# ltdoanh2004/MotionDiffusion-MoE

Hardware: AMD Instinct MI355X
Metric: denoising-steps/sec (B=32, T=196, 263-d, 8 experts) (higher is better)
Workload: dtype bf16; 1 GPU; configs[1]: model_size=small, num_experts=8, B=32/GPU, T=196, 1000-step DDPM with CFG 7.5 (cond+uncond batched as 64 rows), N_text=28, hipGraph=on, streams=1; global_batch=32, parallelism=batch-shard x1, weights replicated

## Files before the change

include/mdm_hip.h:

```cpp
#ifndef MDM_HIP_H
#define MDM_HIP_H
#include <stdint.h>

#ifdef __cplusplus
extern "C" {
#endif

enum { MDM_OK = 0, MDM_ERR_ARG = 1, MDM_ERR_LAUNCH = 2, MDM_ERR_UNSUPPORTED = 3 };
enum { MDM_OP_F32_ROW = 0, MDM_OP_F32_KSTRIDE = 1, MDM_OP_BF16_ROW = 2, MDM_OP_FP8_ROW = 3 ,
       MDM_OP_X2_ROW = 4 };
enum { MDM_ACT_NONE = 0, MDM_ACT_GELU = 1, MDM_ACT_SILU = 2, MDM_ACT_FEAT = 3,
       MDM_ACT_HEADNORM = 4,
       MDM_ACT_HEADSOFTMAX = 5 };
enum { MDM_H16_BF16 = 1, MDM_H16_F16 = 2 };
enum { MDM_PREC_BF16 = 1, MDM_PREC_F16 = 2, MDM_PREC_X3 = 3, MDM_PREC_MIXED = 4, MDM_PREC_FP8 = 5 };

typedef struct MdmOperand {
  const void* p;
  const void* p_lo;
  int64_t ld;
  int64_t gstride;
  const int32_t* gather;
  int64_t bs1, bs2;
  int32_t rpg;
// ... 266 lines not shown

int mdm_motion_fk_max_frames(void);
int mdm_motion_fk(const float* motion, const int32_t* length, const float* mean, const float* std,
                  const MdmSkeleton* skeleton, const float* offsets, int32_t offsets_per_sample, int32_t B, int32_t T,
                  int32_t F, int32_t radius, const double* weights, float* scratch, float* joints_out,
                  float* rotations_out, float* offsets_out, void* stream);

int mdm_foot_skate_max_frames(void);
int mdm_foot_skate(const float* joints, const int32_t* length, const MdmSkeleton* skeleton, const float* contact,
                   int64_t contact_stride, const float* contact_thre, double feet_thre, int32_t blend, int32_t B, int32_t T,
                   const float* rotations_in, float* joints_out, float* rotations_out, float* slide_out, int32_t* pairs_out,
                   float* scratch, void* stream);

enum { MDM_CONTROL_MAX_ITERS = 32 };
int mdm_joint_control_max_frames(int32_t feats);
int mdm_joint_loss_grad(const float* x0, const int32_t* length, const float* mean, const float* std, const float* targets,
                        const float* weights, int32_t B, int32_t T, int32_t F, float* loss_out, float* grad_out,
                        void* stream);
int mdm_joint_guidance(float* x, float* x0, const float* mask, const int32_t* length, const float* mean, const float* std,
                       const float* targets, const float* weights, int32_t B, int32_t T, int32_t F, float scale,
                       int32_t iters, const float* coef, int32_t steps, const int32_t* t_dev, int32_t t_imm,
                       void* stream);

int mdm_handshake_blend(float* x, int32_t groups, int64_t group_stride, int32_t F, int32_t nshared,
                        const int32_t* offsets, const int32_t* rows, const float* weights, void* stream);

typedef struct MdmMoeTensors {
  float* ln_w;
  float* ln_b;
  float* gate_w;
  float* gate_b;
  float* w1;
  float* b1;
  float* w2;
  float* b2;
  float* st_emb_w;
  float* st_emb_b;
  float* st_norm_w;
  float* st_norm_b;
  float* st_out_w;
  float* st_out_b;
} MdmMoeTensors;

int64_t mdm_moe_train_workspace_bytes(int32_t B, int32_t S, int32_t D, int32_t F, int32_t E, int32_t Te);
int mdm_moe_ffn_train_forward(const MdmMoeTensors* params, int32_t D, int32_t F, int32_t E, int32_t Te, int32_t De,
                              const float* eph_w, const float* eph_b, const float* x, const float* emb, int32_t B, int32_t S,
                              float dropout_p, uint64_t seed, float* out, float* lb_loss, int32_t* route_out, void* ws,
                              int64_t ws_bytes, void* stream);
int mdm_moe_ffn_train_backward(const MdmMoeTensors* params, int32_t D, int32_t F, int32_t E, int32_t Te, int32_t De,
                               const float* eph_w, const float* x, const float* emb, int32_t B, int32_t S, float dropout_p,
                               uint64_t seed, const float* dout, float* dx, float* demb, const MdmMoeTensors* grads, void* ws,
                               int64_t ws_bytes, void* stream);
int mdm_sumsq(const float* x, int64_t n, float* out, void* stream);
int mdm_adam_step(float* p, const float* g, float* m, float* v, int64_t n, float lr, float beta1, float beta2, float eps,
                  int32_t step, const float* sumsq, float max_norm, void* stream);

int mdm_xattn_gate(const float* gate, const float* adaptive_gate, int32_t D, float* out, void* stream);
int mdm_fill_i64(int64_t* dst, int64_t n, const int32_t* src_dev, void* stream);
int mdm_add_i32(int32_t* dst, int32_t delta, void* stream);

enum MdmVariant {
  MDM_VAR_DEFAULT = 0,
  MDM_VAR_GEMM_256 = 6,
  MDM_VAR_SD_UNFOLDED = 22,
  MDM_VAR_GENERIC_DH256 = 23,
  MDM_VAR_SD_FOLD_ANY = 24,
  MDM_VAR_ROUTER_CONST_E = 26,
  MDM_VAR_ROUTER_RUNTIME_E = 27,
  MDM_VAR_MLP_LDS = 34,
  MDM_VAR_TAIL_SPLIT = 35,
  MDM_VAR_X3_REG = 36,
  MDM_VAR_QKV_SPLIT = 50,
  MDM_VAR_XQ_SPLIT = 51,
  MDM_VAR_X3_ATTN_CHAIN = 52,
  MDM_VAR_X3_XATTN_CHAIN = 56,
  MDM_VAR_X3_STYLE_SPLIT = 60,
  MDM_VAR_X3_TAILS_SPLIT = 61,
  MDM_VAR_X3_F32_ROWS = 62,
  MDM_VAR_STREAM_NEVER = 63,
  MDM_VAR_STREAM_ALWAYS = 68,
  MDM_VAR_STREAM3_NEVER = 69,
  MDM_VAR_STREAM3_ALWAYS = 70
};
int mdm_set_gemm_variant(int variant);

int mdm_probe_enable(int32_t enable);
int mdm_route_dump(int32_t* buf, int64_t capacity);
int mdm_sd_fold_passes(int32_t D, int32_t H, int32_t N);
int mdm_probe_read(float* us, int32_t* rows, int32_t cap);


int64_t mdm_gru_bidir_workspace_bytes(int32_t B, int32_t H);
int mdm_gru_bidir(const float* gx, const float* w_hh, const float* b_hh, const float* h0, const int32_t* lens_dev,
                  const int32_t* lens_host, int32_t B, int32_t T, int32_t H, float* out, float* ws, int64_t ws_bytes, void* stream);
int mdm_eval_pad_rows(const float* src, int64_t ld_src, int32_t B, int32_t T, int32_t C, int32_t Cp, int32_t pad, int32_t leaky,
                      float* dst, void* stream);
int mdm_eval_ln_leaky(const float* x, int32_t M, int32_t N, const float* w, const float* b, float eps, float* y, void* stream);
int mdm_eval_matching(const float* text, const float* motion, int32_t B, int32_t D, float* dist, int32_t* rank, float* diag,
                      void* stream);
int mdm_eval_center(const float* x, int32_t N, int32_t D, float* mean, float* xc, void* stream);

const char* mdm_version(void);

#ifdef __cplusplus
}
#endif
#endif
```

motiondiffusion-moe_amd/_lib.py:

```python
from __future__ import annotations

import ctypes as C
import os

import torch

_HERE = os.path.dirname(os.path.abspath(__file__))
LIB_PATH = os.environ.get("MDM_LIB") or os.path.join(_HERE, "libmdm_hip.so")
_lib = None

OP_F32_ROW, OP_F32_KSTRIDE, OP_BF16_ROW, OP_FP8_ROW, OP_X2_ROW = 0, 1, 2, 3, 4
ACT_NONE, ACT_GELU, ACT_SILU, ACT_FEAT, ACT_HEADNORM, ACT_HEADSOFTMAX = 0, 1, 2, 3, 4, 5
H16_BF16, H16_F16 = 1, 2
PREC_BF16, PREC_F16, PREC_X3, PREC_MIXED, PREC_FP8 = 1, 2, 3, 4, 5
PRECISIONS = (PREC_BF16, PREC_F16, PREC_X3, PREC_MIXED, PREC_FP8)
PREC_NAMES = {1: "bf16", 2: "f16", 3: "bf16x3(fp32-grade)", 4: "mixed(bf16x3 + f16 expert/FFN GEMMs)",
              5: "f16 + fp8(e4m3) expert GEMMs"}


class MdmError(RuntimeError):
    pass


class Operand(C.Structure):
# ... 46 lines not shown
                ("qkv", Packed), ("qkv_b", C.c_void_p), ("hn_w", C.c_void_p), ("hn_b", C.c_void_p),
                ("feat", Packed), ("proj0", Packed), ("proj3", Packed), ("proj0_b", C.c_void_p),
                ("proj3_b", C.c_void_p), ("proj_ws", C.c_void_p), ("style", Style)]


_P2 = C.c_void_p * 2


class Layer(C.Structure):
    _fields_ = [("dual_pre_w", C.c_void_p), ("dual_pre_b", C.c_void_p), ("dual_post_w", C.c_void_p),
                ("dual_post_b", C.c_void_p), ("local", Performer), ("global_", Performer), ("skip", Packed),
                ("skip_b", C.c_void_p),
                ("ca_norm_w", C.c_void_p), ("ca_norm_b", C.c_void_p), ("ca_tnorm_w", C.c_void_p),
                ("ca_tnorm_b", C.c_void_p), ("ca_q", Packed), ("ca_k", Packed), ("ca_v", Packed),
                ("ca_q_b", C.c_void_p), ("ca_k_b", C.c_void_p), ("ca_v_b", C.c_void_p), ("ca_gvec", C.c_void_p),
                ("ca_style", Style),
                ("moe_ln_w", _P2), ("moe_ln_b", _P2), ("gate_w", _P2), ("gate_b", _P2), ("w1", Packed), ("w2", Packed),
                ("wstream", C.c_void_p), ("wstream_gs", C.c_int64), ("b1", C.c_void_p), ("b2", C.c_void_p), ("usage", _P2), ("importance", _P2), ("ffn_style", Style),
                ("sd_q", Packed), ("sd_k", Packed), ("sd_v", Packed), ("sd_out", Packed), ("sd_f1", Packed),
                ("sd_f2", Packed), ("sd_q_b", C.c_void_p), ("sd_k_b", C.c_void_p), ("sd_v_b", C.c_void_p),
                ("sd_out_b", C.c_void_p), ("sd_ln_w", C.c_void_p), ("sd_ln_b", C.c_void_p), ("sd_f1_b", C.c_void_p),
                ("sd_f2_b", C.c_void_p), ("sd_q_w32", C.c_void_p), ("sd_out_w32", C.c_void_p), ("sd_ffn_ws", C.c_void_p)]


_MODEL_PACKED = ["tmlp0", "tmlp2", "te0", "te2", "tproj", "gf_time", "gf_text", "gf_post0", "gf_post2", "text_proj",
                 "joint", "down", "up", "out"]
_MODEL_BIAS = ["tmlp0_b", "tmlp2_b", "te0_b", "te2_b", "tproj_b", "gf_time_b", "gf_text_b", "gf_post0_b", "gf_post2_b",
               "text_proj_b", "joint_b", "down_b", "up_b2", "out_b"]


class Model(C.Structure):
    _fields_ = ([(n, C.c_int32) for n in ("D", "F", "Dt", "H", "E", "L", "feats", "num_frames")]
                + [(n, Packed) for n in _MODEL_PACKED] + [(n, C.c_void_p) for n in _MODEL_BIAS]
                + [("seq_emb", C.c_void_p), ("style_eph", Packed), ("style_eph_b", C.c_void_p),
                   ("style_emb", Packed), ("style_emb_b", C.c_void_p), ("layers", C.POINTER(Layer))])


SKEL_MAX_JOINTS, SKEL_MAX_CHAINS, SKEL_MAX_CHAIN_ENTRIES = 32, 8, 48


class Skeleton(C.Structure):
    _fields_ = [("joints", C.c_int32), ("nchains", C.c_int32), ("chain_offsets", C.c_int32 * (SKEL_MAX_CHAINS + 1)),
                ("chain_joints", C.c_int32 * SKEL_MAX_CHAIN_ENTRIES), ("raw_offsets", C.c_float * (SKEL_MAX_JOINTS * 3)),
                ("face", C.c_int32 * 4), ("feet", C.c_int32 * 4), ("legs", C.c_int32 * 2)]


class TextCache(C.Structure):
    _fields_ = [("lin_at", C.c_void_p), ("sd_k", C.c_void_p), ("sd_v", C.c_void_p), ("B", C.c_int32),
                ("N", C.c_int32), ("sd_kfold", C.c_void_p), ("sd_cb", C.c_void_p), ("sd_vfold", C.c_void_p),
                ("ntok", C.c_void_p)]


class StemCache(C.Structure):
    _fields_ = [("time_table", C.c_void_p), ("gx", C.c_void_p), ("steps", C.c_int32)]


BLOCK_DUAL, BLOCK_CROSS, BLOCK_MOE, BLOCK_SDCROSS, BLOCK_LAYER = 0, 1, 2, 3, 4
NOISE_STREAM_XT = 0x7FFFFFFF
COMPOSE_MAX_K = 8
CONTROL_MAX_ITERS = 32
TAB_ROWS = 7


def lib():
    global _lib
    if _lib is None:
        if not os.path.exists(LIB_PATH):
            raise MdmError(f"{LIB_PATH} not found: build it with `python motiondiffusion-moe_amd/build.py` "
                           "(hipcc, gfx950). There is no CPU/eager fallback for the denoising path.")
        L = C.CDLL(LIB_PATH)
        L.mdm_version.restype = C.c_char_p
        for name in EXPORTS:
            if name in ("mdm_workspace_bytes", "mdm_text_head_workspace_bytes", "mdm_moe_train_workspace_bytes", "mdm_mlp_stream_elems", "mdm_gemm_stream_elems", "mdm_gemm_stream3_elems", "mdm_gemm_stream1_elems", "mdm_gemm_stream3x_elems", "mdm_gemm_stream3x_group_elems", "mdm_gru_bidir_workspace_bytes"):
                getattr(L, name).restype = C.c_int64
            elif name != "mdm_version":
                getattr(L, name).restype = C.c_int
        _lib = L
    return _lib


EXPORTS = ["mdm_version", "mdm_gemm", "mdm_fused_mlp", "mdm_mlp_stream_elems", "mdm_mlp_stream_pack", "mdm_gemm_stream_elems", "mdm_gemm_stream_pack", "mdm_gemm_stream3_elems", "mdm_gemm_stream3_pack", "mdm_gemm_stream1_elems", "mdm_gemm_stream1_pack", "mdm_gemm_stream3x_elems", "mdm_gemm_stream3x_group_elems", "mdm_gemm_stream3x_pack", "mdm_pack_bf16", "mdm_pack_f16", "mdm_pack_fp8", "mdm_workspace_bytes", "mdm_text_cache_build",
           "mdm_denoiser_forward", "mdm_stem_cache_build", "mdm_block_forward", "mdm_moe_ffn_forward", "mdm_dual_self_attn_forward", "mdm_linear_xattn_forward",
           "mdm_softmax_xattn_ffn_forward", "mdm_performer_attn_forward", "mdm_stylization_forward", "mdm_stem_embeddings",
           "mdm_cfg_posterior_step", "mdm_ddim_step", "mdm_fill_timesteps_mapped", "mdm_guided_update", "mdm_guided_update_inpaint", "mdm_composed_update", "mdm_noise_normal", "mdm_noise_normal_ids", "mdm_text_head_workspace_bytes", "mdm_text_head_forward", "mdm_motion_postprocess", "mdm_motion_features_max_frames", "mdm_motion_features", "mdm_motion_fk_max_frames", "mdm_motion_fk", "mdm_foot_skate_max_frames", "mdm_foot_skate", "mdm_joint_control_max_frames", "mdm_joint_loss_grad", "mdm_joint_guidance", "mdm_handshake_blend", "mdm_xattn_gate", "mdm_fill_i64", "mdm_add_i32", "mdm_set_gemm_variant", "mdm_probe_enable", "mdm_probe_read", "mdm_route_dump",
           "mdm_moe_train_workspace_bytes", "mdm_moe_ffn_train_forward", "mdm_moe_ffn_train_backward", "mdm_sumsq", "mdm_adam_step", "mdm_sd_fold_passes",
           "mdm_gru_bidir_workspace_bytes", "mdm_gru_bidir", "mdm_eval_pad_rows", "mdm_eval_ln_leaky", "mdm_eval_matching", "mdm_eval_center"]


def check(status: int, what: str = "mdm call"):
    if status != 0:
        names = {1: "MDM_ERR_ARG", 2: "MDM_ERR_LAUNCH", 3: "MDM_ERR_UNSUPPORTED"}
        raise MdmError(f"{what} failed: {names.get(status, status)}")


def stream_ptr() -> int:
    return torch.cuda.current_stream().cuda_stream


def ptr(t) -> int:
    return 0 if t is None else t.data_ptr()


def require_cuda(*tensors):
    for t in tensors:
        if t is not None and not t.is_cuda:
            raise MdmError("mdm HIP path needs tensors on a GPU device (no CPU fallback)")
```

motiondiffusion-moe_amd/csrc/api.hip:

```cpp
#include "gemm.h"
#include "kernels.h"

namespace mdm {
namespace {

__global__ void pack_bf16_kernel(const float* __restrict__ src, int64_t ld_src, int64_t rows, int64_t K,
                                 uint16_t* __restrict__ hi, uint16_t* __restrict__ lo, int64_t ld_dst) {
  const int64_t pairs_per_row = ld_dst >> 1;
  const int64_t total = rows * pairs_per_row;
  for (int64_t i = blockIdx.x * (int64_t)blockDim.x + threadIdx.x; i < total; i += (int64_t)gridDim.x * blockDim.x) {
    const int64_t r = i / pairs_per_row, k = (i - r * pairs_per_row) * 2;
    const float a = k < K ? src[r * ld_src + k] : 0.f;
    const float b = k + 1 < K ? src[r * ld_src + k + 1] : 0.f;
    uint32_t h, l;
    split_bf16(a, b, h, l);
    *(uint32_t*)(hi + r * ld_dst + k) = h;
    if (lo) *(uint32_t*)(lo + r * ld_dst + k) = l;
  }
}

__global__ void pack_f16_kernel(const float* __restrict__ src, int64_t ld_src, int64_t rows, int64_t K,
                                uint16_t* __restrict__ dst, int64_t ld_dst) {
  const int64_t pairs_per_row = ld_dst >> 1;
  const int64_t total = rows * pairs_per_row;
  for (int64_t i = blockIdx.x * (int64_t)blockDim.x + threadIdx.x; i < total; i += (int64_t)gridDim.x * blockDim.x) {
    const int64_t r = i / pairs_per_row, k = (i - r * pairs_per_row) * 2;
    const float a = k < K ? src[r * ld_src + k] : 0.f;
    const float b = k + 1 < K ? src[r * ld_src + k + 1] : 0.f;
    *(uint32_t*)(dst + r * ld_dst + k) = pack_f16(a, b);
  }
}

}
}

namespace mdm {
int g_variant = MDM_VAR_DEFAULT;
}

extern "C" {

int mdm_set_gemm_variant(int v) {
  switch (v) {
    case MDM_VAR_DEFAULT:
    case MDM_VAR_GEMM_256:
    case MDM_VAR_SD_UNFOLDED:
    case MDM_VAR_GENERIC_DH256:
    case MDM_VAR_SD_FOLD_ANY:
    case MDM_VAR_ROUTER_CONST_E:
    case MDM_VAR_ROUTER_RUNTIME_E:
    case MDM_VAR_MLP_LDS:
    case MDM_VAR_TAIL_SPLIT:
    case MDM_VAR_X3_REG:
    case MDM_VAR_QKV_SPLIT:
    case MDM_VAR_XQ_SPLIT:
    case MDM_VAR_X3_ATTN_CHAIN:
    case MDM_VAR_X3_XATTN_CHAIN:
    case MDM_VAR_X3_STYLE_SPLIT:
    case MDM_VAR_X3_TAILS_SPLIT:
    case MDM_VAR_X3_F32_ROWS:
    case MDM_VAR_STREAM_NEVER:
    case MDM_VAR_STREAM_ALWAYS:
    case MDM_VAR_STREAM3_NEVER:
    case MDM_VAR_STREAM3_ALWAYS:
      mdm::g_variant = v;
      return MDM_OK;
    default:
      return MDM_ERR_ARG;
  }
}

const char* mdm_version(void) { return "mdm_hip 0.1 (gfx950)"; }

int mdm_gemm(const MdmGemmDesc* d, void* stream) {
  if (!d) return MDM_ERR_ARG;
  return mdm::gemm(*d, (hipStream_t)stream);
}

int mdm_fused_mlp(const MdmMlpDesc* d, void* stream) {
  if (!d) return MDM_ERR_ARG;
  return mdm::fused_mlp(*d, (hipStream_t)stream);
}

int64_t mdm_mlp_stream_elems(int32_t G, int32_t F, int32_t Din, int32_t Dout) { return mdm::mlp_stream_elems(G, F, Din, Dout); }

int mdm_mlp_stream_pack(const float* w1, const float* w2, int32_t G, int32_t F, int32_t Din, int32_t Dout, int32_t h16,
                        uint16_t* out, void* stream) {
  return mdm::mlp_stream_pack(w1, w2, G, F, Din, Dout, h16, out, (hipStream_t)stream);
}

int64_t mdm_gemm_stream_elems(int32_t N, int32_t K) { return mdm::gemm_stream_elems(N, K); }

int mdm_gemm_stream_pack(const float* w, int32_t N, int32_t K, int32_t h16, uint16_t* out, void* stream) {
  return mdm::gemm_stream_pack(w, N, K, h16, out, (hipStream_t)stream);
}

int64_t mdm_gemm_stream1_elems(int32_t N, int32_t K) { return mdm::gemm_stream1_elems(N, K); }

int mdm_gemm_stream1_pack(const float* w, int64_t ldw, int32_t N, int32_t K, int32_t h16, uint16_t* out, void* stream) {
  return mdm::gemm_stream1_pack(w, ldw, N, K, h16, out, (hipStream_t)stream);
}

int64_t mdm_gemm_stream3x_elems(int32_t G, int32_t N, int32_t K) { return mdm::gemm_stream3x_elems(G, N, K); }

int64_t mdm_gemm_stream3x_group_elems(int32_t N, int32_t K) { return mdm::gemm_stream3x_group_elems(N, K); }

int mdm_gemm_stream3x_pack(const float* w, int64_t ldw, int32_t G, int32_t N, int32_t K, uint16_t* out, void* stream) {
  return mdm::gemm_stream3x_pack(w, ldw, G, N, K, out, (hipStream_t)stream);
}

int64_t mdm_gemm_stream3_elems(int32_t N, int32_t K) { return mdm::gemm_stream3_elems(N, K); }

int mdm_gemm_stream3_pack(const float* w, int32_t N, int32_t K, uint16_t* out, void* stream) {
  return mdm::gemm_stream3_pack(w, N, K, out, (hipStream_t)stream);
}

int mdm_pack_bf16(const float* src, int64_t ld_src, int64_t rows, int64_t K, uint16_t* hi, uint16_t* lo,
                  int64_t ld_dst, void* stream) {
  if (!src || !hi || rows < 0 || K <= 0 || ld_dst < K || (ld_dst & 31)) return MDM_ERR_ARG;
  if (rows == 0) return MDM_OK;
  const int64_t total = rows * (ld_dst >> 1);
  int blocks = (int)((total + 255) / 256);
  if (blocks > 4096) blocks = 4096;
  hipLaunchKernelGGL(mdm::pack_bf16_kernel, dim3(blocks), dim3(256), 0, (hipStream_t)stream, src, ld_src, rows, K, hi,
                     lo, ld_dst);
  MDM_RETURN_IF_LAUNCH_FAILED();
  return MDM_OK;
}

int mdm_pack_f16(const float* src, int64_t ld_src, int64_t rows, int64_t K, uint16_t* dst, int64_t ld_dst, void* stream) {
  if (!src || !dst || rows < 0 || K <= 0 || ld_dst < K || (ld_dst & 31)) return MDM_ERR_ARG;
  if (rows == 0) return MDM_OK;
  const int64_t total = rows * (ld_dst >> 1);
  int blocks = (int)((total + 255) / 256);
  if (blocks > 4096) blocks = 4096;
  hipLaunchKernelGGL(mdm::pack_f16_kernel, dim3(blocks), dim3(256), 0, (hipStream_t)stream, src, ld_src, rows, K, dst, ld_dst);
  MDM_RETURN_IF_LAUNCH_FAILED();
  return MDM_OK;
}

int mdm_fill_i64(int64_t* dst, int64_t n, const int32_t* src_dev, void* stream) {
  if (!dst || !src_dev) return MDM_ERR_ARG;
  return mdm::fill_i64(dst, n, src_dev, (hipStream_t)stream);
}

int mdm_add_i32(int32_t* dst, int32_t delta, void* stream) {
  if (!dst) return MDM_ERR_ARG;
// ... 5 lines not shown
```

motiondiffusion-moe_amd/csrc/gemm.h:

```cpp
#pragma once
#include "mdm_common.h"
#include "mdm_hip.h"

namespace mdm {

typedef MdmOperand Operand;
typedef MdmGemmDesc GemmArgs;

enum OperandKind { OP_F32_ROW = MDM_OP_F32_ROW, OP_F32_KSTRIDE = MDM_OP_F32_KSTRIDE, OP_BF16_ROW = MDM_OP_BF16_ROW, OP_X2_ROW = MDM_OP_X2_ROW };
enum Act { ACT_NONE = MDM_ACT_NONE, ACT_GELU = MDM_ACT_GELU, ACT_SILU = MDM_ACT_SILU, ACT_FEAT = MDM_ACT_FEAT, ACT_HEADNORM = MDM_ACT_HEADNORM, ACT_HEADSOFTMAX = MDM_ACT_HEADSOFTMAX };

inline GemmArgs gemm_defaults(int precision) {
  GemmArgs g = {};
  g.batch = 1;
  g.nb2 = 1;
  g.alpha = 1.f;
  g.out_scale = 1.f;
  g.r1_scale = 1.f;
  g.precision = precision;
  g.a_scale_u = 1.f;
  g.c8_scale = 1.f;
  return g;
}
inline Operand op_f32(const float* p, int64_t ld) {
  Operand o = {};
  o.p = p;
  o.ld = ld;
  o.kind = OP_F32_ROW;
  return o;
}
inline Operand op_f32_kstride(const float* p, int64_t ld) {
  Operand o = {};
  o.p = p;
  o.ld = ld;
  o.kind = OP_F32_KSTRIDE;
  return o;
}
inline Operand op_bf16(const uint16_t* hi, const uint16_t* lo, int64_t ld) {
  Operand o = {};
  o.p = hi;
  o.p_lo = lo;
  o.ld = ld;
  o.kind = OP_BF16_ROW;
  return o;
}

int gemm(const GemmArgs& a, hipStream_t stream);
bool gemm_bf16_eligible(const GemmArgs& a);
int gemm_bf16(const GemmArgs& a, hipStream_t stream);
bool gemm_bf16_256_eligible(const GemmArgs& a);
int gemm_bf16_256(const GemmArgs& a, hipStream_t stream);
bool fused_mlp_supported(const MdmMlpDesc& a);
int fused_mlp(const MdmMlpDesc& a, hipStream_t stream);
bool gemm_x3_dma_eligible(const GemmArgs& a);
int gemm_x3_dma(const GemmArgs& a, hipStream_t stream);
bool gemm_fp8_eligible(const GemmArgs& a);
int gemm_fp8(const GemmArgs& a, hipStream_t stream);
int64_t gemm_stream1_elems(int N, int K);
int gemm_stream1_pack(const float* w, int64_t ldw, int N, int K, int h16, uint16_t* out, hipStream_t stream);
bool gemm_stream1_eligible(const GemmArgs& a);
bool gemm_stream1_wanted(const GemmArgs& a);
int gemm_stream1(const GemmArgs& a, hipStream_t stream);
int64_t gemm_stream3x_elems(int G, int N, int K);
int64_t gemm_stream3x_group_elems(int N, int K);
int gemm_stream3x_pack(const float* w, int64_t ldw, int G, int N, int K, uint16_t* out, hipStream_t stream);
bool gemm_stream3x_eligible(const GemmArgs& a);
bool gemm_stream3x_wanted(const GemmArgs& a);
int gemm_stream3x(const GemmArgs& a, hipStream_t stream);
bool fused_mlp_stream_supported(const MdmMlpDesc& a);
int fused_mlp_stream(const MdmMlpDesc& a, hipStream_t stream);
struct PairTail {
  const float *pw, *pb;
  const float *sw, *sb;
  const float* sc;
  int S;
  const uint16_t* ws;
  const float* bias;
  const float* resid;
  float out_scale;
  float* out;
  const float *lw, *lb;
  uint16_t* ln16;
  const float* skip;
  float skip_scale;
  const float *l2w, *l2b;
};
bool fused_pair_style_supported(const MdmMlpDesc& a);
int fused_pair_style(const MdmMlpDesc& a, const PairTail& t, hipStream_t stream);
int64_t mlp_stream_elems(int G, int F, int Din, int Dout);
int mlp_stream_pack(const float* w1, const float* w2, int G, int F, int Din, int Dout, int h16, uint16_t* out, hipStream_t stream);
int64_t gemm_stream_elems(int N, int K);
int gemm_stream_pack(const float* w, int N, int K, int h16, uint16_t* out, hipStream_t stream);
bool style_gemm_supported(int D, int64_t M);
int64_t gemm_stream3_elems(int N, int K);
int gemm_stream3_pack(const float* w, int N, int K, uint16_t* out, hipStream_t stream);
struct StyleTail3 {
  const float *lw = nullptr, *lb = nullptr;
  float* ln_out = nullptr;
  const float* skip = nullptr;
  float skip_scale = 0.f;
  const float *l2w = nullptr, *l2b = nullptr;
  int ln_x2 = 0;
};
int style_gemm3(const float* src, int64_t M, int D, int S, const float* pw, const float* pb, const float* sw, const float* sb,
                const float* sc, const int* pos4, const uint16_t* ws3, const float* bias, const float* resid, float out_scale,
                const float* colscale, float* out, const StyleTail3& t, hipStream_t s);
int style_gemm(const void* src, int src_fmt, int64_t M, int D, int S, const float* pw, const float* pb, const float* sw, const float* sb,
               const float* sc, const int* pos4, const uint16_t* ws, const float* bias, const float* resid, float out_scale,
               const float* colscale, float* out, uint16_t* out16, int h16, hipStream_t s);

}
```

motiondiffusion-moe_amd/csrc/kernels.h:

```cpp
#pragma once
#include "mdm_common.h"

namespace mdm {

enum { TAB_SQRT_RECIP = 0, TAB_SQRT_RECIPM1 = 1, TAB_COEF1 = 2, TAB_COEF2 = 3, TAB_LOGVAR = 4, TAB_ACP = 5,
       TAB_ACP_PREV = 6, TAB_ROWS = 7 };

struct MoeGateParams {
  const float* ln_w[2];
  const float* ln_b[2];
  const float* gate_w[2];
  const float* gate_b[2];
  void* hn;
  int hn_bf16;
  float* hn_scale;
  int* top_idx;
  float* top_val;
  int* hist;
  float* uimp;
  float* usage[2];
  float* importance[2];
  const int* forced_idx;
};

int ln_chain(const float* x, int64_t M, int D, const float* w1, const float* b1, void* y1, int y1_bf, const float* w2,
             const float* b2, void* y2, int y2_bf, hipStream_t s, int x_bf = 0);
int style_in(const float* x, int64_t M, int D, int S, const float* pw, const float* pb, const float* sw,
             const float* sb, const float* sc, const int* pos4, int x_bf, void* out, int out_bf, hipStream_t s);
int to_bf16(const float* src, int64_t n, uint16_t* dst, int h16, hipStream_t s);
int f16_to_bf16x2(const uint16_t* src, int64_t n, uint16_t* hi, uint16_t* lo, hipStream_t s);
int moe_route(const float* x, int64_t M, int D, int E, const MoeGateParams& p, int* goff, int* cursor, int* perm,
              float* rowscale, int* pos4, hipStream_t s);
int head_norm(float* qkv, int64_t M, int H, int dh, const float* w, const float* b, hipStream_t s);
int den_ln(const float* num, const float* phi, int64_t M, int H, int dh, const float* w, const float* b, void* out,
           int out_bf, hipStream_t s);
int head_softmax(float* q, int64_t units, int dh, hipStream_t s);
bool perf_attn_supported(int dh, int S);
bool perf_attn_qkv_supported(int dh, int S, int H);
int perf_attn_qkv(const uint16_t* xn, const uint16_t* wqkv, int ldw, const float* bias, float alpha, uint16_t* qscratch, int h16,
                  const uint16_t* PT, int ldp, const float* hn_w, const float* hn_b, const int* len, int B, int S, int H, int dh,
                  uint16_t* out, hipStream_t s);
int perf_attn(const void* qkv, int h16, const uint16_t* PT, int ldp, const float* hn_w, const float* hn_b, const int* len, int B,
              int S, int H, int dh, uint16_t* out, hipStream_t s);
bool perf_attn256_supported(int dh, int S);
int64_t perf_attn256_scratch_bytes(int B, int H, int S);
int perf_attn256(const void* qkv, int h16, const uint16_t* PT, int ldp, const float* hn_w, const float* hn_b, const int* len,
                 int B, int S, int H, uint16_t* out, void* scratch, hipStream_t s);
bool perf_attn3_supported(int dh, int S);
int perf_attn3(const uint16_t* xh, const uint16_t* xl, const uint16_t* ph, const uint16_t* pl, int ldp, const float* hn_w,
               const float* hn_b, const int* len, int B, int S, int H, int dh, float* out, int out_x2, hipStream_t s);
bool xattn3_supported(int dh, int N);
int lin_xattn3(const uint16_t* qh, const uint16_t* ql, const float* at, int B, int S, int H, int dh, float* out, hipStream_t s);
int sd_attn3(const uint16_t* qh, const uint16_t* ql, const float* kc, const float* vc, const int32_t* ntok, int B, int S, int H,
             int dh, int N, float* out, int out_x2, hipStream_t s);
int row_softmax(float* sc, int64_t rows, int N, hipStream_t s, const int32_t* ntok = nullptr, int64_t rows_per_b = 1);
bool xattn_supported(int dh, int N);
bool lin_xattn_supported(int dh);
int sd_attn(const void* q, int q_fmt, const float* kc, const float* vc, int B, int S, int H, int dh, int N, uint16_t* out16,
            float* out32, int h16, hipStream_t s, const int32_t* ntok = nullptr);
int lin_xattn(const void* ql, int ql_fmt, const float* at, int B, int S, int H, int dh, float* out, uint16_t* out16,
              int h16, hipStream_t s);
bool lin_xattn_q_supported(int dh, int S, int H);
int lin_xattn_q(const uint16_t* xn, const uint16_t* wq, int ldw, const float* bq, const float* at, int B, int S, int H, int dh, float* out,
                uint16_t* out16, int h16, hipStream_t s);
bool sd_fold_supported(int D, int H, int N);
int sd_fold_heads_per_pass(int H, int N);
int sd_fold_passes(int H, int N);
int sd_fold(const uint16_t* x16, const uint16_t* kfold, const float* cb, const uint16_t* vfold, const float* bout,
            const float* ln_w, const float* ln_b, int B, int S, int D, int H, int N, float* out32, uint16_t* out16,
            int h16, hipStream_t s);
int col_softmax(float* k, int B, int N, int D, hipStream_t s, const int32_t* ntok = nullptr);
int sd_fold_mask_cb(float* cb, int B, int np, int hpp, int N, const int32_t* ntok, hipStream_t s);
int sinusoid(const int64_t* t, int B, int D, float* out, hipStream_t s);
int gated_mix(const float* t, const float* x, int64_t n, float* out, hipStream_t s);
int gated_mix_gather(const float* table, const int64_t* ts, int steps, const float* x, int B, int D, float* out,
                     uint16_t* out16, int h16, hipStream_t s);
int text_assemble(const float* pp, const float* ph, int B, int N0, int P, int Dt, float* xf_out, float* xf_proj,
                  hipStream_t s);
int motion_post(const float* x, const int* len, const float* mean, const float* sd, int B, int T, int feats, int J,
                int radius, const double* wts, float* raw, float* out, hipStream_t s);
bool skeleton_ok(const MdmSkeleton& s, int* parent);
int philox_normal(float* out, int64_t per_sample, int nsamples, int64_t sample0, const int64_t* sample_ids, uint64_t seed,
                  const int* stream_dev, int stream_imm, hipStream_t s);
int iota_i64(int64_t* dst, int64_t n, int64_t start, hipStream_t s);
int xattn_gate(const float* gate, const float* ag, int D, float* out, hipStream_t s);
int halve_lengths(const int* len, int B, int* out, hipStream_t s);
int fill_i64(int64_t* dst, int64_t n, const int* src, hipStream_t s);
int add_i32(int* dst, int delta, hipStream_t s);
int cfg_step(const float* x, const float* eps_c, const float* eps_u, const float* noise, int64_t n, const float* tab,
             int ts, const int* t_ptr, int t_imm, float cfg_scale, int clip, float* x_out, float* x0_out, hipStream_t s);
int ddim_step(const float* x, const float* eps, const float* noise, int64_t n, const float* tab, int ts,
              const int* t_ptr, int t_imm, float eta, int clip, float* x_out, float* x0_out, hipStream_t s);

}
```

motiondiffusion-moe_amd/csrc/model.hip:

```cpp
#include "gemm.h"
#include "kernels.h"

namespace mdm {
namespace {

#define MDM_TRY(expr)            \
  do {                           \
    int st__ = (expr);           \
    if (st__ != MDM_OK) return st__; \
  } while (0)

constexpr int PROBE_MAX = 64;
struct Probe {
  bool on = false;
  int n = 0;
  hipEvent_t a[PROBE_MAX], b[PROBE_MAX];
  int rows[PROBE_MAX];
  bool made = false;
};
Probe g_probe;
bool probe_armed() { return g_probe.on && g_probe.n < PROBE_MAX; }
int probe_begin(hipStream_t s) { return probe_armed() && hipEventRecord(g_probe.a[g_probe.n], s) != hipSuccess ? MDM_ERR_LAUNCH : MDM_OK; }
int probe_end(hipStream_t s, int rows) {
  if (!probe_armed()) return MDM_OK;
// ... 115 lines not shown
inline int fmt_mlp(const Ctx& c) { return mlp_x2(c) ? 4 : mlp16(c) ? c.h16 : 0; }

struct Act {
  void* p;
  bool bf;
  bool x2 = false;
};
inline Act act_of(const Ctx& c, float* buf) { return Act{buf, c.bf}; }
inline Act act_x2(const Ctx& c, float* buf) { return Act{buf, c.bf, x2_rows(c)}; }
inline Act act_f32(const float* buf) { return Act{(void*)buf, false}; }
inline Act act_bf16(const uint16_t* buf) { return Act{(void*)buf, true}; }

struct LinOpts {
  int act = ACT_NONE;
  float alpha = 1.f, out_scale = 1.f, r1_scale = 1.f;
  const float* R1 = nullptr;
  const float* R2 = nullptr;
  const float* colscale = nullptr;
  int r1_mod = 0;
  uint16_t* outx2 = nullptr;
};

int linear(const Ctx& c, Act A, int64_t M, int K, const MdmPacked& W, const float* bias, int N, float* out32,
           uint16_t* out16, const LinOpts& o = LinOpts()) {
  GemmArgs g = gd(c);
  if (A.bf) {
    g.A.p = A.p, g.A.ld = K, g.A.kind = OP_BF16_ROW;
    g.precision = 1;
  } else {
    g.A = op_f32((const float*)A.p, K);
    if (A.x2) g.A.kind = OP_X2_ROW;
  }
  g.W = packed(W);
  g.w_stream = A.bf ? W.ws : nullptr;
  g.M = (int)M, g.N = N, g.K = K;
  g.C = out32, g.C16 = out16, g.ldc = N;
  g.Cx2 = o.outx2;
  g.bias = bias;
  g.act = o.act, g.alpha = o.alpha, g.out_scale = o.out_scale;
  g.R1 = o.R1, g.ldr1 = N, g.r1_scale = o.r1_scale, g.r1_mod = o.r1_mod;
  g.R2 = o.R2, g.ldr2 = N;
  g.colscale = o.colscale;
  if (A.bf && !gemm_bf16_eligible(g)) return MDM_ERR_UNSUPPORTED;
  return gemm(g, c.s);
}
int linear_to_act(const Ctx& c, Act A, int64_t M, int K, const MdmPacked& W, const float* bias, int N, float* buf,
                  const LinOpts& o = LinOpts()) {
  return linear(c, A, M, K, W, bias, N, c.bf ? nullptr : buf, c.bf ? (uint16_t*)buf : nullptr, o);
}

inline Operand heads(Operand o, int64_t bs1, int64_t bs2) { o.bs1 = bs1, o.bs2 = bs2; return o; }
GemmArgs per_head(const Ctx& c, Operand A, Operand W, int M, int N, int K, int64_t ldc, int64_t c_bs1, int64_t c_bs2) {
  GemmArgs g = gd(c);
  g.A = A, g.W = W;
  g.M = M, g.N = N, g.K = K;
  g.batch = c.B * c.m->H, g.nb2 = c.m->H;
  g.ldc = ldc, g.c_bs1 = c_bs1, g.c_bs2 = c_bs2;
  return g;
}

GemmArgs planes_gemm(const Ctx& c, Act A, const MdmPacked& W, const float* bias, int N, uint16_t* hi, uint16_t* lo) {
  const int K = c.m->D;
  GemmArgs g = gd(c);
  g.A = op_f32((const float*)A.p, K);
  if (A.x2) g.A.kind = OP_X2_ROW;
  g.W = packed(W);
  g.M = (int)c.M, g.N = N, g.K = K;
  g.bias = bias;
  g.C16 = hi, g.C16_lo = lo, g.ldc = N;
  return g;
}

enum class StylePath { FUSED16, FUSED3, FUSED3_TAIL, SPLIT };
StylePath style_path(const Ctx& c, const MdmStyle& st, bool src16, bool out16, bool tail) {
  const int D = c.m->D;
  if (c.bf && st.out_ws && style_gemm_supported(D, c.M)) return StylePath::FUSED16;
  if (x3_flow(c) && !src16 && !out16 && st.out_ws3 && g_variant != MDM_VAR_X3_STYLE_SPLIT && style_gemm_supported(D, c.M))
    return tail && g_variant != MDM_VAR_X3_TAILS_SPLIT ? StylePath::FUSED3_TAIL : StylePath::FUSED3;
  return StylePath::SPLIT;
}

int style_apply(const Ctx& c, const MdmStyle& st, const float* src, const float* pw, const float* pb, const int* pos4,
                const float* sc, float* tmp, const float* resid, float out_scale, const float* colscale, float* out,
                uint16_t* out16 = nullptr, bool src_bf16 = false, const StyleTail3* t3 = nullptr) {
  const int D = c.m->D;
  const StylePath path = style_path(c, st, src_bf16, out16 != nullptr, t3 != nullptr);
  switch (path) {
    case StylePath::FUSED16:
      return style_gemm(src, src_bf16 ? c.h16 : 0, c.M, D, c.S, pw, pb, st.norm_w, st.norm_b, sc, pos4, st.out_ws, st.out_b, resid,
                        out_scale, colscale, out, out16, c.h16, c.s);
    case StylePath::FUSED3:
    case StylePath::FUSED3_TAIL:
      return style_gemm3(src, c.M, D, c.S, pw, pb, st.norm_w, st.norm_b, sc, pos4, st.out_ws3, st.out_b, resid, out_scale, colscale, out,
                         path == StylePath::FUSED3_TAIL ? *t3 : StyleTail3(), c.s);
    case StylePath::SPLIT: {
      MDM_TRY(style_in(src, c.M, D, c.S, pw, pb, st.norm_w, st.norm_b, sc, pos4, src_bf16 ? c.h16 : 0, tmp, fmt16(c), c.s));
      LinOpts o;
      o.out_scale = out_scale, o.R1 = resid, o.colscale = colscale;
      return linear(c, act_of(c, tmp), c.M, D, st.out, st.out_b, D, out, out16, o);
    }
  }
}

MdmMlpDesc proj_pair_desc(const Ctx& c, const MdmPerformer& p) {
  const int D = c.m->D;
  MdmMlpDesc f = {};
  f.X = (const uint16_t*)c.w.t4, f.ldx = D, f.M = (int)c.M, f.Din = D, f.F = D, f.Dout = D;
  f.b1 = p.proj0_b, f.b2 = p.proj3_b, f.wstream = p.proj_ws, f.wstream_gs = 2 * (int64_t)D * D;
  f.r1_scale = 1.f, f.C16 = (uint16_t*)c.w.t4, f.ldc = D, f.h16 = c.h16;
  return f;
}
enum class ProjPath { PAIR_TAIL, PAIR, LINEARS_X2, LINEARS };
ProjPath proj_path(const Ctx& c, const MdmPerformer& p) {
  if (c.bf && p.proj_ws) {
    const MdmMlpDesc f = proj_pair_desc(c, p);
    if (p.style.out_ws && g_variant != MDM_VAR_TAIL_SPLIT && fused_pair_style_supported(f)) return ProjPath::PAIR_TAIL;
    if (fused_mlp_stream_supported(f)) return ProjPath::PAIR;
  }
  return x2_rows(c) ? ProjPath::LINEARS_X2 : ProjPath::LINEARS;
}

enum class PerfCore { CORE3, CORE256, CORE16_QKV, CORE16, CHAIN };
PerfCore perf_core_path(const Ctx& c, const MdmPerformer& p, bool xn16) {
  const int D = c.m->D, H = c.m->H, dh = D / H;
  if (c.bf && g_variant != MDM_VAR_GENERIC_DH256 && perf_attn256_supported(dh, c.S) &&
      perf_attn256_scratch_bytes(c.B, H, c.S) <= c.M * 2 * D * (int64_t)sizeof(float))
    return PerfCore::CORE256;
  if (c.bf && perf_attn_supported(dh, c.S))
    return xn16 && g_variant != MDM_VAR_QKV_SPLIT && perf_attn_qkv_supported(dh, c.S, H) ? PerfCore::CORE16_QKV : PerfCore::CORE16;
  if (x3_flow(c) && !xn16 && g_variant != MDM_VAR_X3_ATTN_CHAIN && perf_attn3_supported(dh, c.S) && D % 32 == 0 && p.qkv.lo &&
      p.feat.lo && (c.M * 3 * D) % 8 == 0)
    return PerfCore::CORE3;
  return PerfCore::CHAIN;
}

int performer(const Ctx& c, const MdmPerformer& p, const float* x, Act xn, const float* sc, float* out,
              const StyleTail3& pt = StyleTail3()) {
  const MdmModel& m = *c.m;
  const int D = m.D, H = m.H, dh = D / H, mf = dh;
  const Work& w = c.w;
  LinOpts qo;
  qo.alpha = 0.1f;
  Act att = act_of(c, w.t4);
  switch (perf_core_path(c, p, xn.bf)) {
    case PerfCore::CORE3: {
      uint16_t* const xh = (uint16_t*)w.qkv;
      uint16_t* const xl = xh + c.M * 3 * D;
      GemmArgs g = planes_gemm(c, xn, p.qkv, p.qkv_b, 3 * D, xh, xl);
      g.alpha = 0.1f, g.act = ACT_HEADNORM, g.hn_w = p.hn_w, g.hn_b = p.hn_b, g.hn_l2_tiles = 2 * H;
      MDM_TRY(gemm(g, c.s));
      MDM_TRY(perf_attn3(xh, xl, p.feat.hi, p.feat.lo, (int)p.feat.ld, p.hn_w, p.hn_b, c.len, c.B, c.S, H, dh, w.t4, c.x2 ? 1 : 0, c.s));
      att.x2 = c.x2;
      break;
    }
    case PerfCore::CORE256:
      MDM_TRY(linear(c, xn, c.M, D, p.qkv, p.qkv_b, 3 * D, nullptr, (uint16_t*)w.qkv, qo));
      MDM_TRY(perf_attn256(w.qkv, c.h16, p.feat.hi, (int)p.feat.ld, p.hn_w, p.hn_b, c.len, c.B, c.S, H, (uint16_t*)w.t4, w.phi, c.s));
      break;
    case PerfCore::CORE16_QKV:
      MDM_TRY(perf_attn_qkv((const uint16_t*)xn.p, p.qkv.hi, (int)p.qkv.ld, p.qkv_b, 0.1f, (uint16_t*)w.qkv, c.h16, p.feat.hi,
                            (int)p.feat.ld, p.hn_w, p.hn_b, c.len, c.B, c.S, H, dh, (uint16_t*)w.t4, c.s));
      break;
    case PerfCore::CORE16:
      MDM_TRY(linear(c, xn, c.M, D, p.qkv, p.qkv_b, 3 * D, nullptr, (uint16_t*)w.qkv, qo));
      MDM_TRY(perf_attn(w.qkv, c.h16, p.feat.hi, (int)p.feat.ld, p.hn_w, p.hn_b, c.len, c.B, c.S, H, dh, (uint16_t*)w.t4, c.s));
      break;
    case PerfCore::CHAIN: {
      MDM_TRY(linear(c, xn, c.M, D, p.qkv, p.qkv_b, 3 * D, w.qkv, nullptr, qo));
      MDM_TRY(head_norm(w.qkv, c.M, H, dh, p.hn_w, p.hn_b, c.s));
      const bool f16p = c.bf && c.h16 == MDM_H16_F16 && !p.feat.lo;
      Operand P = packed(p.feat);
      if (f16p) {
        const int64_t pn = (int64_t)mf * p.feat.ld;
// ... 33 lines not shown
      t.ws = p.style.out_ws, t.bias = p.style.out_b, t.resid = x, t.out_scale = 0.1f, t.out = out;
      t.lw = pt.lw, t.lb = pt.lb, t.ln16 = (uint16_t*)pt.ln_out, t.skip = pt.skip, t.skip_scale = pt.skip_scale, t.l2w = pt.l2w, t.l2b = pt.l2b;
      return fused_pair_style(proj_pair_desc(c, p), t, c.s);
    }
    case ProjPath::PAIR:
      MDM_TRY(fused_mlp_stream(proj_pair_desc(c, p), c.s));
      break;
    case ProjPath::LINEARS_X2: {
      LinOpts o;
      o.act = ACT_GELU, o.outx2 = (uint16_t*)w.t2;
      MDM_TRY(linear(c, att, c.M, D, p.proj0, p.proj0_b, D, nullptr, nullptr, o));
      MDM_TRY(linear(c, Act{w.t2, false, true}, c.M, D, p.proj3, p.proj3_b, D, w.t4, nullptr));
      break;
    }
    case ProjPath::LINEARS: {
      LinOpts o;
      o.act = ACT_GELU;
      MDM_TRY(linear_to_act(c, att, c.M, D, p.proj0, p.proj0_b, D, w.t2, o));
      MDM_TRY(linear_to_act(c, act_of(c, w.t2), c.M, D, p.proj3, p.proj3_b, D, w.t4));
      break;
    }
  }
  const bool tail3 = !c.bf && (pt.ln_out || pt.skip);
  return style_apply(c, p.style, w.t4, p.post_w, p.post_b, nullptr, sc, w.t2, x, 0.1f, nullptr, out, nullptr, c.bf,
                     tail3 ? &pt : nullptr);
}

enum class DualTail { NONE, T16, T3 };
DualTail dual_tail_path(const Ctx& c, const MdmLayer& l) {
  if (proj_path(c, l.local) == ProjPath::PAIR_TAIL && proj_path(c, l.global) == ProjPath::PAIR_TAIL) return DualTail::T16;
  if (style_path(c, l.local.style, false, false, true) == StylePath::FUSED3_TAIL &&
      style_path(c, l.global.style, false, false, true) == StylePath::FUSED3_TAIL)
    return DualTail::T3;
  return DualTail::NONE;
}

int dual_block(const Ctx& c, const MdmLayer& l, const float* x, const uint16_t* x16, const float* sc4, float* out,
               const float* next_w = nullptr, const float* next_b = nullptr) {
  const int D = c.m->D;
  const Work& w = c.w;
  const int64_t scs = (int64_t)c.B * 2 * D;
  const int xnf = fmt_xn(c);
  const Act xa = c.bf ? act_bf16(x16) : act_f32(x);
  LinOpts so;
  so.act = ACT_GELU;
  switch (dual_tail_path(c, l)) {
    case DualTail::T16:
    case DualTail::T3: {
      MDM_TRY(linear(c, xa, c.M, D, l.skip, l.skip_b, D, w.f1, nullptr, so));
      MDM_TRY(ln_chain(x, c.M, D, l.dual_pre_w, l.dual_pre_b, w.t1, 0, l.local.pre_w, l.local.pre_b, w.t3, xnf, c.s));
      StyleTail3 pt;
      pt.lw = l.global.pre_w, pt.lb = l.global.pre_b, pt.ln_out = w.t3, pt.ln_x2 = c.x2;
      MDM_TRY(performer(c, l.local, w.t1, act_x2(c, w.t3), sc4 + 0 * scs, w.t5, pt));
      StyleTail3 bt;
      bt.skip = w.f1, bt.skip_scale = 0.1f, bt.lw = l.dual_post_w, bt.lb = l.dual_post_b;
      if (next_w) bt.l2w = next_w, bt.l2b = next_b, bt.ln_out = w.t2, bt.ln_x2 = c.x2;
      return performer(c, l.global, w.t5, act_x2(c, w.t3), sc4 + 1 * scs, out, bt);
    }
    case DualTail::NONE: {
      MDM_TRY(ln_chain(x, c.M, D, l.dual_pre_w, l.dual_pre_b, w.t1, 0, l.local.pre_w, l.local.pre_b, w.t3, xnf, c.s));
      const bool normed = proj_path(c, l.local) == ProjPath::PAIR_TAIL;
      StyleTail3 pt;
      if (normed) pt.lw = l.global.pre_w, pt.lb = l.global.pre_b, pt.ln_out = w.t3;
      MDM_TRY(performer(c, l.local, w.t1, act_x2(c, w.t3), sc4 + 0 * scs, w.t5, pt));
      if (!normed) MDM_TRY(ln_chain(w.t5, c.M, D, l.global.pre_w, l.global.pre_b, w.t3, xnf, nullptr, nullptr, nullptr, 0, c.s));
      MDM_TRY(performer(c, l.global, w.t5, act_x2(c, w.t3), sc4 + 1 * scs, w.t1));
      so.R1 = w.t1, so.r1_scale = 0.1f;
      MDM_TRY(linear(c, xa, c.M, D, l.skip, l.skip_b, D, w.t3, nullptr, so));
      return ln_chain(w.t3, c.M, D, l.dual_post_w, l.dual_post_b, out, 0, next_w, next_b, next_w ? w.t2 : nullptr, xnf, c.s);
    }
  }
}

enum class XattnPath { CORE3, CORE_Q, CORE, CHAIN };
XattnPath lin_xattn_path(const Ctx& c, const MdmLayer& l) {
  const int D = c.m->D, H = c.m->H, dh = D / H;
  if (c.bf && lin_xattn_supported(dh) && !(dh == 256 && g_variant == MDM_VAR_GENERIC_DH256))
    return g_variant != MDM_VAR_XQ_SPLIT && D == 512 && lin_xattn_q_supported(dh, c.S, H) ? XattnPath::CORE_Q : XattnPath::CORE;
  if (x3_flow(c) && g_variant != MDM_VAR_X3_XATTN_CHAIN && xattn3_supported(dh, 1) && l.ca_q.lo && D % 32 == 0 && (c.M * D) % 8 == 0)
    return XattnPath::CORE3;
  return XattnPath::CHAIN;
}

int cross_block(const Ctx& c, const MdmLayer& l, const float* at, const float* x, const float* sc, float* out,
                bool pre_normed = false) {
  const MdmModel& m = *c.m;
  const int D = m.D, H = m.H, dh = D / H;
  const Work& w = c.w;
  if (!pre_normed) MDM_TRY(ln_chain(x, c.M, D, l.ca_norm_w, l.ca_norm_b, w.t2, fmt_xn(c), nullptr, nullptr, nullptr, 0, c.s));
  bool y16 = false;
  switch (lin_xattn_path(c, l)) {
    case XattnPath::CORE3: {
      uint16_t* const qh = (uint16_t*)w.t3;
      uint16_t* const ql = qh + c.M * D;
      GemmArgs g = planes_gemm(c, act_x2(c, w.t2), l.ca_q, l.ca_q_b, D, qh, ql);
      g.act = ACT_HEADSOFTMAX;
      MDM_TRY(gemm(g, c.s));
      MDM_TRY(lin_xattn3(qh, ql, at, c.B, c.S, H, dh, w.t4, c.s));
      break;
    }
    case XattnPath::CORE_Q:
      MDM_TRY(lin_xattn_q((const uint16_t*)w.t2, l.ca_q.hi, (int)l.ca_q.ld, l.ca_q_b, at, c.B, c.S, H, dh, nullptr, (uint16_t*)w.t4,
                          c.h16, c.s));
      y16 = true;
      break;
    case XattnPath::CORE:
      MDM_TRY(linear(c, act_x2(c, w.t2), c.M, D, l.ca_q, l.ca_q_b, D, nullptr, (uint16_t*)w.t3));
      MDM_TRY(lin_xattn(w.t3, c.h16, at, c.B, c.S, H, dh, nullptr, (uint16_t*)w.t4, c.h16, c.s));
      y16 = true;
      break;
    case XattnPath::CHAIN: {
      MDM_TRY(linear(c, act_x2(c, w.t2), c.M, D, l.ca_q, l.ca_q_b, D, w.t3, nullptr));
      MDM_TRY(head_softmax(w.t3, c.M * H, dh, c.s));
      GemmArgs g = per_head(c, heads(op_f32(w.t3, D), (int64_t)c.S * D, dh), heads(op_f32(at, dh), (int64_t)H * dh * dh, (int64_t)dh * dh),
                            c.S, dh, dh, D, (int64_t)c.S * D, dh);
      g.C = w.t4;
      MDM_TRY(gemm(g, c.s));
      break;
    }
  }
  return style_apply(c, l.ca_style, w.t4, nullptr, nullptr, nullptr, sc, w.t2, x, 1.f, l.ca_gvec, out, nullptr, y16);
}

GemmArgs expert_gemm(const Ctx& c, const void* A, int K, const MdmPacked& W, const float* bias, int N) {
  GemmArgs g = gd(c);
  if (c.fp8) {
    g.A.p = A, g.A.ld = K, g.A.kind = MDM_OP_FP8_ROW;
    g.W.p = W.hi, g.W.ld = W.ld, g.W.kind = MDM_OP_FP8_ROW, g.w_scale = (const float*)W.lo;
  } else if (mlp16(c)) {
    g.A.p = A, g.A.ld = K, g.A.kind = OP_BF16_ROW, g.precision = 1;
    g.W = packed(W);
  } else {
    g.A = op_f32((const float*)A, K);
    if (mlp_x2(c)) g.A.kind = OP_X2_ROW;
    g.W = packed(W);
  }
  g.W.bs1 = (int64_t)N * W.ld;
  g.goff = c.w.goff, g.ngroups = 2 * c.m->E;
  g.M = (int)(4 * c.M), g.N = N, g.K = K;
  g.bias = bias, g.bias_bs = N;
  g.ldc = N;
  if (mlp_x2(c) && W.ws) g.w_stream = W.ws, g.w_stream_gs = gemm_stream3x_group_elems(N, K);
  return g;
}
enum class MoePath { FP8, FUSED, GROUPED };
MoePath moe_path(const Ctx& c, const MdmMlpDesc& f) {
  if (c.fp8) return MoePath::FP8;
  return mlp16(c) && fused_mlp_supported(f) ? MoePath::FUSED : MoePath::GROUPED;
}

int moe_block(const Ctx& c, const MdmLayer& l, const float* x, const float* sc, const int* forced, float* out,
              uint16_t* out16, int32_t* route_out = nullptr) {
  const MdmModel& m = *c.m;
  const int D = m.D, F = m.F, E = m.E;
  const Work& w = c.w;
  MoeGateParams p = {};
  for (int b = 0; b < 2; ++b) {
    p.ln_w[b] = l.moe_ln_w[b], p.ln_b[b] = l.moe_ln_b[b];
    p.gate_w[b] = l.gate_w[b], p.gate_b[b] = l.gate_b[b];
    p.usage[b] = l.usage[b], p.importance[b] = l.importance[b];
  }
  p.hn = w.hn, p.hn_bf16 = c.fp8 ? 3 : fmt_mlp(c), p.hn_scale = w.hn_scale, p.top_idx = w.top_idx, p.top_val = w.top_val, p.hist = w.hist, p.uimp = w.uimp, p.forced_idx = forced;
  MDM_TRY(moe_route(x, c.M, D, E, p, w.goff, w.cursor, w.perm, w.rowscale, w.pos4, c.s));
  if (route_out && hipMemcpyAsync(route_out, w.top_idx, 4 * c.M * sizeof(int32_t), hipMemcpyDeviceToDevice, c.s) != hipSuccess)
    return MDM_ERR_LAUNCH;
  MdmMlpDesc f = {};
  f.X = (const uint16_t*)w.hn, f.ldx = D, f.gather = w.perm;
  f.M = (int)(4 * c.M), f.Din = D, f.F = F, f.Dout = D;
  f.goff = w.goff, f.ngroups = 2 * E;
  f.w1 = l.w1.hi, f.ldw1 = l.w1.ld, f.w1_gs = (int64_t)F * l.w1.ld, f.b1 = l.b1, f.b1_gs = F;
  f.w2 = l.w2.hi, f.ldw2 = l.w2.ld, f.w2_gs = (int64_t)D * l.w2.ld, f.b2 = l.b2, f.b2_gs = D;
  f.rowscale = w.rowscale, f.r1_scale = 1.f;
  f.C = w.y2, f.ldc = D;
  f.h16 = c.h16;
  f.wstream = l.wstream, f.wstream_gs = l.wstream_gs;
  switch (moe_path(c, f)) {
    case MoePath::FP8: {
      const float HS = 8.f;
      GemmArgs g1 = expert_gemm(c, w.hn, D, l.w1, l.b1, F);
      g1.A.gather = w.perm, g1.a_scale = w.hn_scale, g1.act = ACT_GELU, g1.C8 = (uint8_t*)w.hid, g1.c8_scale = HS;
      MDM_TRY(gemm(g1, c.s));
      GemmArgs g2 = expert_gemm(c, w.hid, F, l.w2, l.b2, D);
      g2.a_scale_u = 1.f / HS, g2.rowscale = w.rowscale, g2.C16 = (uint16_t*)w.y2;
      MDM_TRY(gemm(g2, c.s));
      return style_apply(c, l.ffn_style, w.y2, nullptr, nullptr, w.pos4, sc, w.t2, x, 1.f, nullptr, out, out16, true);
    }
    case MoePath::FUSED: {
      if (c.bf) f.C = nullptr, f.C16 = (uint16_t*)w.y2;
      MDM_TRY(probe_begin(c.s));
      MDM_TRY(fused_mlp(f, c.s));
      MDM_TRY(probe_end(c.s, f.M));
      return style_apply(c, l.ffn_style, w.y2, nullptr, nullptr, w.pos4, sc, w.t2, x, 1.f, nullptr, out, out16, c.bf);
    }
    case MoePath::GROUPED: {
      MDM_TRY(probe_begin(c.s));
      GemmArgs g1 = expert_gemm(c, w.hn, D, l.w1, l.b1, F);
      g1.A.gather = w.perm, g1.act = ACT_GELU;
      if (mlp16(c)) g1.C16 = (uint16_t*)w.hid;
      else if (mlp_x2(c)) g1.Cx2 = (uint16_t*)w.hid;
      else g1.C = w.hid;
      MDM_TRY(gemm(g1, c.s));
      GemmArgs g2 = expert_gemm(c, w.hid, F, l.w2, l.b2, D);
      g2.rowscale = w.rowscale, g2.C = w.y2;
      MDM_TRY(gemm(g2, c.s));
      MDM_TRY(probe_end(c.s, (int)(4 * c.M)));
      return style_apply(c, l.ffn_style, w.y2, nullptr, nullptr, w.pos4, sc, w.t2, x, 1.f, nullptr, out, out16, false);
    }
  }
}

int sd_fold_policy(int D, int H, int N) {
  if (!sd_fold_supported(D, H, N)) return 0;
  const int np = sd_fold_passes(H, N);
  return (np <= 2 || g_variant == MDM_VAR_SD_FOLD_ANY) ? np : 0;
}

struct SdFold {
  const uint16_t* kfold = nullptr;
  const float* cb = nullptr;
  const uint16_t* vfold = nullptr;
};

enum class SdPath { FOLD_PAIR, FOLD, CORE3, CORE, CHAIN };
SdPath sd_path(const Ctx& c, const MdmLayer& l, const SdFold& fold, const MdmMlpDesc& f) {
  const int D = c.m->D, H = c.m->H, dh = D / H, N = c.N;
  if (c.bf && fold.kfold && g_variant != MDM_VAR_SD_UNFOLDED && sd_fold_policy(D, H, N) > 0)
    return l.sd_ffn_ws && c.S >= 128 && fused_mlp_stream_supported(f) ? SdPath::FOLD_PAIR : SdPath::FOLD;
  if (x3_flow(c) && g_variant != MDM_VAR_X3_XATTN_CHAIN && xattn3_supported(dh, N) && l.sd_q.lo && D % 32 == 0 && (c.M * D) % 8 == 0)
    return SdPath::CORE3;
  if (c.bf && xattn_supported(dh, N) && !(dh == 256 && g_variant == MDM_VAR_GENERIC_DH256)) return SdPath::CORE;
  return SdPath::CHAIN;
}

int sd_ffn(const Ctx& c, const MdmLayer& l, const float* x, float* out, uint16_t* out16) {
  const int D = c.m->D;
  const Work& w = c.w;
  const bool h = mlp16(c), x2 = mlp_x2(c);
  LinOpts o1;
  o1.act = ACT_GELU;
  if (x2) o1.outx2 = (uint16_t*)w.f1;
  MDM_TRY(linear(c, Act{w.t4, h, x2}, c.M, D, l.sd_f1, l.sd_f1_b, 4 * D, (h || x2) ? nullptr : w.f1, h ? (uint16_t*)w.f1 : nullptr, o1));
  LinOpts o;
  o.R1 = x, o.R2 = w.t3;
  return linear(c, Act{w.f1, h, x2}, c.M, 4 * D, l.sd_f2, l.sd_f2_b, D, out, out16, o);
}

// ... 6 lines not shown
  f.X = (const uint16_t*)w.t4, f.ldx = D, f.M = (int)c.M, f.Din = D, f.F = 4 * D, f.Dout = D;
  f.b1 = l.sd_f1_b, f.b2 = l.sd_f2_b, f.wstream = l.sd_ffn_ws, f.wstream_gs = 8 * (int64_t)D * D;
  f.R1 = x, f.ldr1 = D, f.r1_scale = 1.f, f.R2 = w.t3, f.ldr2 = D;
  f.C = out, f.C16 = out16, f.ldc = D, f.h16 = c.h16;
  const SdPath path = sd_path(c, l, fold, f);
  const Act xa = c.bf ? act_bf16(x16) : act_f32(x);
  LinOpts qo;
  qo.alpha = 1.f / sqrtf((float)dh);
  Act att = act_of(c, w.t2);
  switch (path) {
    case SdPath::FOLD_PAIR:
    case SdPath::FOLD:
      MDM_TRY(sd_fold(x16, fold.kfold, fold.cb, fold.vfold, l.sd_out_b, l.sd_ln_w, l.sd_ln_b, c.B, c.S, D, H, N, w.t3,
                      (uint16_t*)w.t4, c.h16, c.s));
      return path == SdPath::FOLD_PAIR ? fused_mlp_stream(f, c.s) : sd_ffn(c, l, x, out, out16);
    case SdPath::CORE3: {
      uint16_t* const qh = (uint16_t*)w.t1;
      uint16_t* const ql = qh + c.M * D;
      GemmArgs g = planes_gemm(c, act_f32(x), l.sd_q, l.sd_q_b, D, qh, ql);
      g.alpha = qo.alpha;
      MDM_TRY(gemm(g, c.s));
      MDM_TRY(sd_attn3(qh, ql, kc, vc, c.ntok, c.B, c.S, H, dh, N, w.t2, c.x2 ? 1 : 0, c.s));
      att.x2 = c.x2;
      break;
    }
    case SdPath::CORE:
      MDM_TRY(linear(c, xa, c.M, D, l.sd_q, l.sd_q_b, D, nullptr, (uint16_t*)w.t1, qo));
      MDM_TRY(sd_attn(w.t1, c.h16, kc, vc, c.B, c.S, H, dh, N, (uint16_t*)w.t2, nullptr, c.h16, c.s, c.ntok));
      break;
    case SdPath::CHAIN: {
      MDM_TRY(linear(c, xa, c.M, D, l.sd_q, l.sd_q_b, D, w.t1, nullptr, qo));
      GemmArgs g = per_head(c, heads(op_f32(w.t1, D), (int64_t)c.S * D, dh), heads(op_f32(kc, D), (int64_t)N * D, dh), c.S, N, dh,
                            N, (int64_t)H * c.S * N, (int64_t)c.S * N);
      g.C = w.scr;
      MDM_TRY(gemm(g, c.s));
      MDM_TRY(row_softmax(w.scr, c.M * H, N, c.s, c.ntok, (int64_t)H * c.S));
      GemmArgs pv = per_head(c, heads(op_f32(w.scr, N), (int64_t)H * c.S * N, (int64_t)c.S * N),
                             heads(op_f32_kstride(vc, D), (int64_t)N * D, dh), c.S, dh, N, D, (int64_t)c.S * D, dh);
      pv.C = c.bf ? nullptr : w.t2, pv.C16 = c.bf ? (uint16_t*)w.t2 : nullptr;
      MDM_TRY(gemm(pv, c.s));
      break;
    }
  }
  MDM_TRY(linear(c, att, c.M, D, l.sd_out, l.sd_out_b, D, w.t3, nullptr));
  MDM_TRY(ln_chain(w.t3, c.M, D, l.sd_ln_w, l.sd_ln_b, w.t4, fmt_mlp(c), nullptr, nullptr, nullptr, 0, c.s));
  return sd_ffn(c, l, x, out, out16);
}

const float* tc_at(const MdmModel& m, const MdmTextCache& tc, int layer) {
  const int dh = m.D / m.H;
  return tc.lin_at + (int64_t)layer * tc.B * m.H * dh * dh;
}
const float* tc_k(const MdmModel& m, const MdmTextCache& tc, int layer) {
  return tc.sd_k + (int64_t)layer * tc.B * tc.N * m.D;
}
const float* tc_v(const MdmModel& m, const MdmTextCache& tc, int layer) {
  return tc.sd_v + (int64_t)layer * tc.B * tc.N * m.D;
}
SdFold tc_fold(const MdmModel& m, const MdmTextCache& tc, int layer) {
  SdFold f;
  if (tc.sd_kfold && tc.sd_cb && tc.sd_vfold) {
    const int64_t np = sd_fold_passes(m.H, tc.N);
    f.kfold = tc.sd_kfold + (int64_t)layer * tc.B * np * 128 * m.D;
    f.cb = tc.sd_cb + (int64_t)layer * tc.B * np * 128;
    f.vfold = tc.sd_vfold + (int64_t)layer * tc.B * np * m.D * 128;
  }
  return f;
}

int decoder_layer(const Ctx& c, int layer, const MdmTextCache& tc, float* x, uint16_t* x16, float* y, uint16_t* y16,
                  const float* sc4, const int* forced, float* trace, int32_t* route_out = nullptr) {
  const MdmModel& m = *c.m;
  const MdmLayer& l = m.layers[layer];
  const int64_t scs = (int64_t)c.B * 2 * m.D, n = c.M * m.D;
  auto dump = [&](int slot, const float* p) -> int {
    if (!trace) return MDM_OK;
    return hipMemcpyAsync(trace + (int64_t)slot * n, p, n * sizeof(float), hipMemcpyDeviceToDevice, c.s) == hipSuccess
               ? MDM_OK
               : MDM_ERR_LAUNCH;
  };
  if (!c.bf) x16 = y16 = nullptr;
  MDM_TRY(dual_block(c, l, x, x16, sc4, y, l.ca_norm_w, l.ca_norm_b));
  MDM_TRY(dump(0, y));
  MDM_TRY(cross_block(c, l, tc_at(m, tc, layer), y, sc4 + 2 * scs, x, true));
  MDM_TRY(dump(1, x));
  MDM_TRY(moe_block(c, l, x, sc4 + 3 * scs, forced, y, y16, route_out));
  MDM_TRY(dump(2, y));
  MDM_TRY(sdcross_block(c, l, tc_k(m, tc, layer), tc_v(m, tc, layer), y, y16, x, x16, tc_fold(m, tc, layer)));
  return dump(3, x);
}

int stem_time_branch(const Ctx& c, const int64_t* timesteps, int B, float* dst) {
  const MdmModel& m = *c.m;
  const int D = m.D, Te = 4 * D;
  const Work& w = c.w;
  LinOpts silu_o;
  silu_o.act = ACT_SILU;
  MDM_TRY(sinusoid(timesteps, B, D, w.s_a, c.s));
  MDM_TRY(linear(c, act_f32(w.s_a), B, D, m.tmlp0, m.tmlp0_b, 2 * D, w.s_b, nullptr, silu_o));
  MDM_TRY(linear(c, act_f32(w.s_b), B, 2 * D, m.tmlp2, m.tmlp2_b, D, w.s_a, nullptr));
  MDM_TRY(linear(c, act_f32(w.s_a), B, D, m.te0, m.te0_b, Te, w.s_b, nullptr, silu_o));
  MDM_TRY(linear(c, act_f32(w.s_b), B, Te, m.te2, m.te2_b, Te, w.s_c, nullptr));
  MDM_TRY(linear(c, act_f32(w.s_c), B, Te, m.tproj, m.tproj_b, D, w.s_a, nullptr));
  return linear(c, act_f32(w.s_a), B, D, m.gf_time, m.gf_time_b, D, dst, nullptr);
}

int stem_text_branch(const Ctx& c, const float* xf_proj, int B, float* dst) {
  const MdmModel& m = *c.m;
  const float* tp = xf_proj;
  if (m.Dt != m.D) {
    if (!m.text_proj.hi) return MDM_ERR_ARG;
    MDM_TRY(linear(c, act_f32(xf_proj), B, m.Dt, m.text_proj, m.text_proj_b, m.D, c.w.s_c, nullptr));
    tp = c.w.s_c;
  }
  return linear(c, act_f32(tp), B, m.D, m.gf_text, m.gf_text_b, m.D, dst, nullptr);
}

int stem_embeddings(const Ctx& c, const int64_t* timesteps, const float* xf_proj, const MdmStemCache* sc_cache,
                    float* emb_out, float* sc_out) {
  const MdmModel& m = *c.m;
  const int D = m.D, Te = 4 * D, B = c.B, nblk = 8 * m.L;
  const Work& w = c.w;
  LinOpts silu_o;
  silu_o.act = ACT_SILU;
  float* mix = w.s_b;
  if (sc_cache && sc_cache->time_table && sc_cache->gx) {
    MDM_TRY(gated_mix_gather(sc_cache->time_table, timesteps, sc_cache->steps, sc_cache->gx, B, D, c.bf ? nullptr : mix,
                             c.bf ? (uint16_t*)mix : nullptr, c.h16, c.s));
  } else {
    MDM_TRY(stem_time_branch(c, timesteps, B, w.s_b));
    MDM_TRY(stem_text_branch(c, xf_proj, B, w.s_a));
    MDM_TRY(gated_mix(w.s_b, w.s_a, (int64_t)B * D, w.s_c, c.s));
    if (c.bf) {
      MDM_TRY(to_bf16(w.s_c, (int64_t)B * D, (uint16_t*)w.s_b, c.h16, c.s));
    } else {
      mix = w.s_c;
    }
  }
  MDM_TRY(linear_to_act(c, act_of(c, mix), B, D, m.gf_post0, m.gf_post0_b, D, w.s_a, silu_o));
  float* emb = emb_out ? emb_out : w.emb;
  MDM_TRY(linear(c, act_of(c, w.s_a), B, D, m.gf_post2, m.gf_post2_b, D, emb, c.bf ? (uint16_t*)w.s_c : nullptr));
  MDM_TRY(linear_to_act(c, c.bf ? act_bf16((uint16_t*)w.s_c) : act_f32(emb), B, D, m.style_eph, m.style_eph_b, nblk * Te,
                        w.e1, silu_o));
  GemmArgs g = gd(c);
  if (c.bf) {
    g.A.p = w.e1, g.A.ld = (int64_t)nblk * Te, g.A.kind = OP_BF16_ROW, g.precision = 1;
  } else {
    g.A = op_f32(w.e1, (int64_t)nblk * Te);
  }
  g.A.bs1 = Te;
  g.W = packed(m.style_emb);
  g.W.bs1 = (int64_t)2 * D * m.style_emb.ld;
  g.M = B, g.N = 2 * D, g.K = Te;
  g.batch = nblk, g.nb2 = 1;
  g.bias = m.style_emb_b, g.bias_bs = 2 * D;
  g.C = sc_out, g.ldc = 2 * D, g.c_bs1 = (int64_t)B * 2 * D;
  return gemm(g, c.s);
}

int check_model(const MdmModel* m) {
  if (!m || !m->layers || m->D <= 0 || m->H <= 0 || m->D % m->H || m->L <= 0 || m->E < 2 || m->E > 16) return MDM_ERR_ARG;
  const int dh = m->D / m->H;
  if (dh != 16 && dh != 32 && dh != 64 && dh != 128 && dh != 256) return MDM_ERR_UNSUPPORTED;
  if (m->D > 1024 || m->Dt > 1024 || (m->D & 3) || (m->F & 3)) return MDM_ERR_UNSUPPORTED;
  return MDM_OK;
}

}
}
// ... 239 lines not shown
                                  int64_t ws_bytes, int32_t precision, void* stream) {
  return mdm_block_forward(m, layer, MDM_BLOCK_SDCROSS, tc, h, sc4, len, B, S, out, ws, ws_bytes, nullptr, precision, stream);
}
int mdm_performer_attn_forward(const MdmModel* m, int32_t layer, int32_t which, const float* h, const float* sc,
                               const int32_t* len, int32_t B, int32_t S, float* out, void* ws, int64_t ws_bytes,
                               int32_t precision, void* stream) {
  MDM_TRY(check_model(m));
  if (!h || !sc || !len || !out || !ws || B <= 0 || S <= 0 || layer < 0 || layer >= 2 * m->L || which < 0 || which > 1)
    return MDM_ERR_ARG;
  Ctx c = {};
  c.m = m, c.s = (hipStream_t)stream, c.B = B, c.S = S, c.M = (int64_t)B * S, c.len = len, c.N = 1;
  if (!set_precision(c, m, precision)) return MDM_ERR_UNSUPPORTED;
  c.w = carve(*m, B, S, 1, ws);
  if (c.w.bytes > ws_bytes) return MDM_ERR_ARG;
  const MdmLayer& l = m->layers[layer];
  const MdmPerformer& p = which ? l.global : l.local;
  MDM_TRY(ln_chain(h, c.M, m->D, p.pre_w, p.pre_b, c.w.t3, fmt16(c), nullptr, nullptr, nullptr, 0, c.s));
  return performer(c, p, h, act_of(c, c.w.t3), sc, out);
}

int mdm_stylization_forward(const MdmStyle* st, const float* h, const float* sc, int32_t B, int32_t S, int32_t D,
                            float* tmp, float* out, int32_t precision, void* stream) {
  if (!st || !h || !sc || !tmp || !out || B <= 0 || S <= 0) return MDM_ERR_ARG;
  MdmModel fake = {};
  fake.D = D;
  Ctx c = {};
  fake.F = D;
  c.m = &fake, c.s = (hipStream_t)stream, c.B = B, c.S = S, c.M = (int64_t)B * S;
  if (!set_precision(c, &fake, precision)) return MDM_ERR_UNSUPPORTED;
  return style_apply(c, *st, h, nullptr, nullptr, nullptr, sc, tmp, nullptr, 1.f, nullptr, out);
}

int64_t mdm_text_head_workspace_bytes(int32_t B, int32_t N0, int32_t P, int32_t Hs, int32_t Dt) {
  if (B <= 0 || N0 < 0 || P < 0 || Hs <= 0 || Dt <= 0) return -1;
  const int64_t fl = (int64_t)B * N0 * Hs + (int64_t)P * Hs + (int64_t)B * N0 * Dt + (int64_t)P * Dt;
  return ((fl * 4 + 255) & ~(int64_t)255) + 1024;
}

int mdm_text_head_forward(const float* hidden, const float* prompts, const float* ln_w, const float* ln_b,
                          const MdmPacked* w, const float* bias, int32_t B, int32_t N0, int32_t P, int32_t Hs,
                          int32_t Dt, float* xf_out, float* xf_proj, void* ws, int64_t ws_bytes, int32_t precision,
                          void* stream) {
  if (!ln_w || !ln_b || !w || !w->hi || !xf_out || !xf_proj || !ws || B <= 0 || N0 < 0 || P < 0 || N0 + P <= 0 ||
      (N0 > 0 && !hidden) || (P > 0 && !prompts))
    return MDM_ERR_ARG;
  if (precision != 1 && precision != 3) return MDM_ERR_ARG;
  if (precision == 3 && !w->lo) return MDM_ERR_ARG;
  if (ws_bytes < mdm_text_head_workspace_bytes(B, N0, P, Hs, Dt)) return MDM_ERR_ARG;
  hipStream_t s = (hipStream_t)stream;
  Bump b(ws);
  float* lnh = b.take<float>((int64_t)B * N0 * Hs);
  float* lnp = b.take<float>((int64_t)P * Hs);
  float* ph = b.take<float>((int64_t)B * N0 * Dt);
  float* pp = b.take<float>((int64_t)P * Dt);
  MdmModel fake = {};
  Ctx c = {};
  c.m = &fake, c.s = s, c.prec = precision, c.bf = false, c.mix = false, c.h16 = MDM_H16_BF16;
  LinOpts o;
  o.act = ACT_GELU;
  if (N0 > 0) {
    MDM_TRY(ln_chain(hidden, (int64_t)B * N0, Hs, ln_w, ln_b, lnh, 0, nullptr, nullptr, nullptr, 0, s));
    MDM_TRY(linear(c, act_f32(lnh), (int64_t)B * N0, Hs, *w, bias, Dt, ph, nullptr, o));
  }
  if (P > 0) {
    MDM_TRY(ln_chain(prompts, P, Hs, ln_w, ln_b, lnp, 0, nullptr, nullptr, nullptr, 0, s));
    MDM_TRY(linear(c, act_f32(lnp), P, Hs, *w, bias, Dt, pp, nullptr, o));
  }
  return text_assemble(pp, ph, B, N0, P, Dt, xf_out, xf_proj, s);
}

int mdm_motion_postprocess(const float* motion, const int32_t* length, const float* mean, const float* std, int32_t B,
                           int32_t T, int32_t feats, int32_t joints, int32_t radius, const double* weights,
                           float* scratch, float* joints_out, void* stream) {
  if (!motion || !mean || !std || !scratch || !joints_out || B <= 0 || T <= 0 || joints < 1 || radius < 0 ||
      (radius > 0 && !weights))
    return MDM_ERR_ARG;
  if (feats < 4 + 3 * (joints - 1)) return MDM_ERR_ARG;
  return motion_post(motion, length, mean, std, B, T, feats, joints, radius, weights, scratch, joints_out,
                     (hipStream_t)stream);
}

int mdm_sd_fold_passes(int32_t D, int32_t H, int32_t N) { return sd_fold_policy(D, H, N); }

int mdm_route_dump(int32_t* buf, int64_t capacity) {
  if (buf && capacity <= 0) return MDM_ERR_ARG;
  g_route_dump = buf, g_route_cap = buf ? capacity : 0;
  return MDM_OK;
}

int mdm_probe_enable(int32_t enable) {
  if (enable && !g_probe.made) {
    for (int i = 0; i < PROBE_MAX; ++i)
      if (hipEventCreate(&g_probe.a[i]) != hipSuccess || hipEventCreate(&g_probe.b[i]) != hipSuccess) return MDM_ERR_LAUNCH;
    g_probe.made = true;
  }
  g_probe.on = enable != 0;
  if (enable) g_probe.n = 0;
  return MDM_OK;
}

int mdm_probe_read(float* us, int32_t* rows, int32_t cap) {
  const int n = g_probe.n;
  for (int i = 0; i < n && i < cap; ++i) {
    if (hipEventSynchronize(g_probe.b[i]) != hipSuccess) return -1;
    float ms = 0.f;
    if (hipEventElapsedTime(&ms, g_probe.a[i], g_probe.b[i]) != hipSuccess) return -1;
    if (us) us[i] = ms * 1e3f;
    if (rows) rows[i] = g_probe.rows[i];
  }
  return n;
}

int mdm_cfg_posterior_step(const float* x, const float* eps_c, const float* eps_u, const float* noise, int64_t n,
                           const float* tab, int32_t steps, const int32_t* t_dev, int32_t t_imm, float cfg_scale,
                           int32_t clip_denoised, float* x_out, float* x0_out, void* stream) {
  if (steps <= 0 || (!t_dev && (t_imm < 0 || t_imm >= steps))) return MDM_ERR_ARG;
  return cfg_step(x, eps_c, eps_u, noise, n, tab, steps, t_dev, t_imm, cfg_scale, clip_denoised, x_out, x0_out,
                  (hipStream_t)stream);
}

int mdm_ddim_step(const float* x, const float* eps, const float* noise, int64_t n, const float* tab, int32_t steps,
                  const int32_t* t_dev, int32_t t_imm, float eta, int32_t clip_denoised, float* x_out, float* x0_out,
                  void* stream) {
  if (steps <= 0 || (!t_dev && (t_imm < 0 || t_imm >= steps))) return MDM_ERR_ARG;
  return ddim_step(x, eps, noise, n, tab, steps, t_dev, t_imm, eta, clip_denoised, x_out, x0_out, (hipStream_t)stream);
}

int mdm_xattn_gate(const float* gate, const float* adaptive_gate, int32_t D, float* out, void* stream) {
  if (!gate || !adaptive_gate || !out || D <= 0) return MDM_ERR_ARG;
  return xattn_gate(gate, adaptive_gate, D, out, (hipStream_t)stream);
}

}
```

motiondiffusion-moe_amd/csrc/rowwise.hip:

```cpp
#include "kernels.h"
#include "row.h"

namespace mdm {
namespace {

template <int NE, bool VEC, int FMT>
__device__ __forceinline__ void ln_chain_rows(const float* __restrict__ x, bool x_h, int64_t M, int D, const float* w1,
                                              const float* b1, void* y1, int y1_h, const float* w2, const float* b2,
                                              void* y2, int y2_h) {
  const int lane = threadIdx.x & 63;
  Row<NE, VEC> ww1, bb1, ww2, bb2;
  ww1.load(w1, D, lane), bb1.load(b1, D, lane);
  if (w2) ww2.load(w2, D, lane), bb2.load(b2, D, lane);
  for (int64_t row = 2 * (blockIdx.x * (int64_t)WPB + (threadIdx.x >> 6)); row < M; row += 2 * (int64_t)gridDim.x * WPB) {
    const bool two = row + 1 < M;
    Row<NE, VEC> r, q;
    if (x_h) {
      r.template load_h16<FMT>((const uint16_t*)x + row * D, D, lane);
      q.template load_h16<FMT>((const uint16_t*)x + (two ? row + 1 : row) * D, D, lane);
    } else {
      r.load(x + row * D, D, lane);
      q.load(x + (two ? row + 1 : row) * D, D, lane);
    }
    r.layernorm(ww1, bb1, D, lane);
    q.layernorm(ww1, bb1, D, lane);
    if (y1) {
      r.template store_mode<FMT>(y1, row, D, lane, y1_h);
      if (two) q.template store_mode<FMT>(y1, row + 1, D, lane, y1_h);
    }
    if (w2) {
      r.layernorm(ww2, bb2, D, lane);
      q.layernorm(ww2, bb2, D, lane);
      r.template store_mode<FMT>(y2, row, D, lane, y2_h);
      if (two) q.template store_mode<FMT>(y2, row + 1, D, lane, y2_h);
    }
  }
}
template <int NE, bool VEC>
__global__ __launch_bounds__(256) void ln_chain_kernel(const float* __restrict__ x, int x_bf, int64_t M, int D,
                                                       const float* w1, const float* b1, void* y1, int y1_bf,
                                                       const float* w2, const float* b2, void* y2, int y2_bf) {
  const int m1 = y1_bf == 4 ? 2 : (y1_bf != 0), m2 = y2_bf == 4 ? 2 : (y2_bf != 0);
  if (((x_bf | y1_bf | y2_bf) & 3) == 2) {
    ln_chain_rows<NE, VEC, 2>(x, x_bf != 0, M, D, w1, b1, y1, m1, w2, b2, y2, m2);
  } else {
    ln_chain_rows<NE, VEC, 1>(x, x_bf != 0, M, D, w1, b1, y1, m1, w2, b2, y2, m2);
  }
}

template <int NE, bool VEC, int FMT>
__device__ __forceinline__ void style_in_rows(const float* __restrict__ x, int64_t M, int D, int S, const float* pw,
                                              const float* pb, const float* sw, const float* sb,
                                              const float* __restrict__ sc, const int* __restrict__ pos4, bool x_h,
                                              void* __restrict__ out, bool out_h) {
  const int lane = threadIdx.x & 63;
  Row<NE, VEC> pww, pbb, sww, sbb;
  if (pw) pww.load(pw, D, lane), pbb.load(pb, D, lane);
  sww.load(sw, D, lane), sbb.load(sb, D, lane);
  for (int64_t row = blockIdx.x * (int64_t)WPB + (threadIdx.x >> 6); row < M; row += (int64_t)gridDim.x * WPB) {
    const float* scb = sc + (row / S) * 2 * (int64_t)D;
    Row<NE, VEC> r, scale, shift;
    scale.load(scb, D, lane);
    shift.load(scb + D, D, lane);
    if (pos4) {
      const int p0 = pos4[row * 4 + 0], p1 = pos4[row * 4 + 1], p2 = pos4[row * 4 + 2], p3 = pos4[row * 4 + 3];
      Row<NE, VEC> a, b, c, d;
      if (x_h) {
        const uint16_t* xh = (const uint16_t*)x;
        a.template load_h16<FMT>(xh + (int64_t)p0 * D, D, lane);
        b.template load_h16<FMT>(xh + (int64_t)p1 * D, D, lane);
        c.template load_h16<FMT>(xh + (int64_t)p2 * D, D, lane);
        d.template load_h16<FMT>(xh + (int64_t)p3 * D, D, lane);
      } else {
        a.load(x + (int64_t)p0 * D, D, lane);
        b.load(x + (int64_t)p1 * D, D, lane);
        c.load(x + (int64_t)p2 * D, D, lane);
        d.load(x + (int64_t)p3 * D, D, lane);
      }
#pragma unroll
      for (int j = 0; j < NE; ++j) r.e[j] = ((a.e[j] + b.e[j]) + (c.e[j] + d.e[j])) * 0.5f;
    } else {
      if (x_h) {
        r.template load_h16<FMT>((const uint16_t*)x + row * D, D, lane);
// ... 92 lines not shown
              v2 = pe, i2 = e;
            }
          }
        }
        if (!(v2 >= 0.f)) {
          i2 = i1 == 0 ? 1 : 0;
          v1 = v2 = __int_as_float(0x7fc00000);
        }
      }
      if (lane == 0) {
        const int64_t o = ((int64_t)br * M + row) * 2;
        p.top_idx[o] = i1, p.top_idx[o + 1] = i2;
        p.top_val[o] = v1, p.top_val[o + 1] = v2;
        atomicAdd(&s_hist[br * E + i1], 1);
        atomicAdd(&s_hist[br * E + i2], 1);
        atomicAdd(&s_usage[br * E + i1], 1.f);
        atomicAdd(&s_imp[br * E + i1], v1);
        atomicAdd(&s_imp[br * E + i2], v2);
      }
    }
  }
  __syncthreads();
  if (threadIdx.x < 2 * E) {
    const int g = threadIdx.x;
    p.hist[blockIdx.x * 32 + g] = s_hist[g];
    p.uimp[blockIdx.x * 64 + g] = s_usage[g];
    p.uimp[blockIdx.x * 64 + 32 + g] = s_imp[g];
  }
}

template <int NV, bool FAST, int EX = 0, int HNF = -1>
__global__ __launch_bounds__(256) void moe_gate16_kernel(const float* __restrict__ x, int64_t M, int D_rt, int E_rt,
                                                         MoeGateParams p) {
  const int E = EX > 0 ? EX : E_rt;
  const int hnf = HNF >= 0 ? HNF : p.hn_bf16;
  constexpr int D = 64 * NV;
  extern __shared__ __attribute__((aligned(16))) float gsm[];
  float* gw = gsm;
  float* lnw = gsm + 2 * E * D;
  float* lnb = lnw + 2 * D;
  int* s_hist = (int*)(lnb + 2 * D);
  float* s_usage = (float*)(s_hist + 32);
  float* s_imp = s_usage + 32;
  const int l16 = threadIdx.x & 15;
  const int64_t tpb = 16;
  const int64_t stride = (int64_t)gridDim.x * tpb;
  auto load_x = [&](int64_t base, f32x4(&r)[NV]) {
    const int64_t row = base + (threadIdx.x >> 4);
    const int64_t rc = row < M ? row : M - 1;
#pragma unroll
    for (int c = 0; c < NV; ++c) r[c] = *(const f32x4*)(x + rc * D + 4 * (l16 + 16 * c));
  };
  f32x4 vn[NV];
  if constexpr (NV <= 8)
    if (blockIdx.x * tpb < M) load_x(blockIdx.x * tpb, vn);
#pragma unroll
  for (int br = 0; br < 2; ++br) {
    const float* src = p.gate_w[br];
    const int n4 = E * D / 4;
    for (int i0 = threadIdx.x; i0 < n4; i0 += 4 * 256) {
      f32x4 t[4];
#pragma unroll
      for (int j = 0; j < 4; ++j)
        if (i0 + 256 * j < n4) t[j] = *(const f32x4*)(src + 4 * (i0 + 256 * j));
#pragma unroll
      for (int j = 0; j < 4; ++j)
        if (i0 + 256 * j < n4) *(f32x4*)(gw + br * E * D + 4 * (i0 + 256 * j)) = t[j];
    }
  }
  for (int i = threadIdx.x; i < D / 4; i += 256) {
    const f32x4 w0 = *(const f32x4*)(p.ln_w[0] + 4 * i), w1 = *(const f32x4*)(p.ln_w[1] + 4 * i);
    const f32x4 b0 = *(const f32x4*)(p.ln_b[0] + 4 * i), b1 = *(const f32x4*)(p.ln_b[1] + 4 * i);
    *(f32x4*)(lnw + 4 * i) = w0, *(f32x4*)(lnw + D + 4 * i) = w1;
    *(f32x4*)(lnb + 4 * i) = b0, *(f32x4*)(lnb + D + 4 * i) = b1;
  }
  if (threadIdx.x < 32) s_hist[threadIdx.x] = 0, s_usage[threadIdx.x] = 0.f, s_imp[threadIdx.x] = 0.f;
  __syncthreads();
  for (int64_t base = blockIdx.x * tpb; base < M; base += stride) {
    const int64_t row = base + (threadIdx.x >> 4);
    const bool ok = row < M;
    const int64_t rc = ok ? row : M - 1;
    if constexpr (NV > 8) load_x(base, vn);
    f32x4 v[NV];
    float s = 0.f;
#pragma unroll
    for (int c = 0; c < NV; ++c) {
      v[c] = vn[c];
      s += v[c][0] + v[c][1] + v[c][2] + v[c][3];
    }
    if constexpr (NV <= 8)
      if (base + stride < M) load_x(base + stride, vn);
    const float mean = group_sum<16>(s) / D;
    float q = 0.f;
#pragma unroll
    for (int c = 0; c < NV; ++c) {
      v[c] = (f32x4){v[c][0] - mean, v[c][1] - mean, v[c][2] - mean, v[c][3] - mean};
      q += v[c][0] * v[c][0] + v[c][1] * v[c][1] + v[c][2] * v[c][2] + v[c][3] * v[c][3];
    }
    const float rstd = rsqrtf(group_sum<16>(q) / D + 1e-5f);
#pragma unroll
    for (int br = 0; br < 2; ++br) {
      float logit[16];
#pragma unroll
      for (int e = 0; e < 16; ++e) logit[e] = 0.f;
      float amax = 0.f;
#pragma unroll
      for (int c = 0; c < NV; ++c) {
        const int k = 4 * (l16 + 16 * c);
        const f32x4 w = *(const f32x4*)(lnw + br * D + k), b = *(const f32x4*)(lnb + br * D + k);
        const f32x4 h = {v[c][0] * rstd * w[0] + b[0], v[c][1] * rstd * w[1] + b[1], v[c][2] * rstd * w[2] + b[2],
                         v[c][3] * rstd * w[3] + b[3]};
        amax = fmaxf(amax, fmaxf(fmaxf(fabsf(h[0]), fabsf(h[1])), fmaxf(fabsf(h[2]), fabsf(h[3]))));
        if constexpr (HNF >= 0) {
          if constexpr (HNF == 1 || HNF == 2) {
            *(uint2*)((uint16_t*)p.hn + ((int64_t)br * M + rc) * D + k) = make_uint2(pack_h16(HNF, h[0], h[1]), pack_h16(HNF, h[2], h[3]));
          } else if constexpr (HNF == 0) {
            *(f32x4*)((float*)p.hn + ((int64_t)br * M + rc) * D + k) = h;
          } else if constexpr (HNF == 4) {
            static_assert(D % 32 == 0, "lane pairs of store_x2_4p hold k and k ^ 4 of one 32-column block");
            store_x2_4p((uint16_t*)p.hn + ((int64_t)br * M + rc) * 2 * D, k, h[0], h[1], h[2], h[3]);
          }
        } else if (ok && p.hn_bf16 != 3) {
          if (p.hn_bf16 == 4) {
            store_x2_4((uint16_t*)p.hn + ((int64_t)br * M + row) * 2 * D, k, h[0], h[1], h[2], h[3]);
          } else if (p.hn_bf16 == 2) {
            *(uint2*)((uint16_t*)p.hn + ((int64_t)br * M + row) * D + k) = make_uint2(pack_h16(2, h[0], h[1]), pack_h16(2, h[2], h[3]));
          } else if (p.hn_bf16) {
            *(uint2*)((uint16_t*)p.hn + ((int64_t)br * M + row) * D + k) = make_uint2(pack_h16(1, h[0], h[1]), pack_h16(1, h[2], h[3]));
          } else {
            *(f32x4*)((float*)p.hn + ((int64_t)br * M + row) * D + k) = h;
          }
        }
#pragma unroll
        for (int e = 0; e < 16; ++e)
          if (e < E) {
            const f32x4 g = *(const f32x4*)(gw + (br * E + e) * D + k);
            if constexpr (FAST) {
              logit[e] = __builtin_fmaf(h[3], g[3], __builtin_fmaf(h[2], g[2], __builtin_fmaf(h[1], g[1], __builtin_fmaf(h[0], g[0], logit[e]))));
            } else {
              logit[e] += h[0] * g[0] + h[1] * g[1] + h[2] * g[2] + h[3] * g[3];
            }
          }
        if constexpr (EX > 0 && HNF >= 0) __builtin_amdgcn_sched_barrier(0);
      }
      if (hnf == 3) {
        amax = group_max<16>(amax);
        const float scale = amax > 0.f ? amax * (1.f / 448.f) : 1.f, inv = 1.f / scale;
#pragma unroll
        for (int c = 0; c < NV; ++c) {
          const int k = 4 * (l16 + 16 * c);
          const f32x4 w = *(const f32x4*)(lnw + br * D + k), b = *(const f32x4*)(lnb + br * D + k);
          uint32_t q = 0;
          q = __builtin_amdgcn_cvt_pk_fp8_f32((v[c][0] * rstd * w[0] + b[0]) * inv, (v[c][1] * rstd * w[1] + b[1]) * inv, q, false);
          q = __builtin_amdgcn_cvt_pk_fp8_f32((v[c][2] * rstd * w[2] + b[2]) * inv, (v[c][3] * rstd * w[3] + b[3]) * inv, q, true);
          if (HNF >= 0 || ok) *(uint32_t*)((uint8_t*)p.hn + ((int64_t)br * M + (HNF >= 0 ? rc : row)) * D + k) = q;
        }
        if (ok && l16 == 0) p.hn_scale[(int64_t)br * M + row] = scale;
      }
      float mx = -INFINITY, mine = -INFINITY;
#pragma unroll
      for (int e = 0; e < 16; ++e) {
        if (e < E) {
          logit[e] = group_sum<16>(logit[e]) + p.gate_b[br][e];
          mx = fmaxf(mx, logit[e]);
          mine = (l16 == e) ? logit[e] : mine;
        }
      }
      const float den = group_sum<16>(l16 < E ? expf(mine - mx) : 0.f);
      int i1 = 0, i2 = 1;
      float l1 = -INFINITY, l2 = -INFINITY;
      if (p.forced_idx) {
        i1 = min(max(p.forced_idx[((int64_t)br * M + rc) * 2 + 0], 0), E - 1);
        i2 = min(max(p.forced_idx[((int64_t)br * M + rc) * 2 + 1], 0), E - 1);
#pragma unroll
        for (int e = 0; e < 16; ++e) {
          l1 = e == i1 ? logit[e] : l1;
          l2 = e == i2 ? logit[e] : l2;
        }
      } else {
#pragma unroll
        for (int e = 0; e < 16; ++e) {
          if (e < E) {
            if (logit[e] > l1) {
              l2 = l1, i2 = i1;
              l1 = logit[e], i1 = e;
            } else if (logit[e] > l2) {
              l2 = logit[e], i2 = e;
            }
          }
        }
        if (i2 == i1) i2 = i1 == 0 ? 1 : 0;
      }
      const float v1 = expf(l1 - mx) / den, v2 = expf(l2 - mx) / den;
      if (ok && l16 == 0) {
        const int64_t o = ((int64_t)br * M + row) * 2;
        p.top_idx[o] = i1, p.top_idx[o + 1] = i2;
        p.top_val[o] = v1, p.top_val[o + 1] = v2;
        atomicAdd(&s_hist[br * E + i1], 1);
        atomicAdd(&s_hist[br * E + i2], 1);
        atomicAdd(&s_usage[br * E + i1], 1.f);
        atomicAdd(&s_imp[br * E + i1], v1);
        atomicAdd(&s_imp[br * E + i2], v2);
      }
    }
  }
  __syncthreads();
  if (threadIdx.x < 2 * E) {
    const int g = threadIdx.x;
    p.hist[blockIdx.x * 32 + g] = s_hist[g];
    p.uimp[blockIdx.x * 64 + g] = s_usage[g];
    p.uimp[blockIdx.x * 64 + 32 + g] = s_imp[g];
  }
}

__global__ __launch_bounds__(1024) void moe_offsets_kernel(const int* __restrict__ hist_part,
                                                            const float* __restrict__ uimp_part, int nparts, int E,
                                                            int* __restrict__ goff, int* __restrict__ cursor,
                                                            MoeGateParams p) {
  __shared__ int sh[32][33];
  __shared__ float su[32][33], si[32][33];
  __shared__ int tot[32];
  const int g = threadIdx.x & 31, c = threadIdx.x >> 5, G = 2 * E;
  int h = 0;
  float u = 0.f, im = 0.f;
  if (g < G) {
#pragma unroll 4
    for (int b = c; b < nparts; b += 32) {
      h += hist_part[b * 32 + g];
      u += uimp_part[b * 64 + g];
      im += uimp_part[b * 64 + 32 + g];
    }
  }
  sh[c][g] = h, su[c][g] = u, si[c][g] = im;
  __syncthreads();
  if (threadIdx.x < G) {
    int ht = 0;
    float ut = 0.f, it = 0.f;
    for (int k = 0; k < 32; ++k) ht += sh[k][g], ut += su[k][g], it += si[k][g];
    tot[g] = ht;
    cursor[g] = 0;
    const int br = g / E, e = g - br * E;
    if (p.usage[br]) {
      atomicAdd(&p.usage[br][e], ut);
      atomicAdd(&p.importance[br][e], it);
    }
  }
  __syncthreads();
  if (threadIdx.x == 0) {
    int s = 0;
    for (int i = 0; i < G; ++i) {
      goff[i] = s;
      s += tot[i];
    }
    goff[G] = s;
  }
}

__global__ __launch_bounds__(256) void moe_assign_kernel(const int* __restrict__ top_idx, const float* __restrict__ top_val,
                                                         int64_t M, int E, const int* __restrict__ goff,
                                                         int* __restrict__ cursor, int* __restrict__ perm,
                                                         float* __restrict__ rowscale, int* __restrict__ pos4) {
  __shared__ int s_cnt[32], s_base[32];
  const int64_t total = 2 * M * 2;
  for (int64_t base = blockIdx.x * (int64_t)blockDim.x; base < total; base += (int64_t)gridDim.x * blockDim.x) {
    if (threadIdx.x < 32) s_cnt[threadIdx.x] = 0;
    __syncthreads();
    const int64_t i = base + threadIdx.x;
    int g = -1, rank = 0;
    int64_t br = 0, tok = 0;
    int k = 0;
    if (i < total) {
      br = i / (2 * M);
      const int64_t rem = i - br * 2 * M;
      tok = rem >> 1, k = (int)(rem & 1);
      g = (int)br * E + min(max(top_idx[i], 0), E - 1);
      rank = atomicAdd(&s_cnt[g], 1);
    }
    __syncthreads();
    if (threadIdx.x < 2 * E && s_cnt[threadIdx.x]) s_base[threadIdx.x] = atomicAdd(&cursor[threadIdx.x], s_cnt[threadIdx.x]);
    __syncthreads();
    if (g >= 0) {
      const int pos = goff[g] + s_base[g] + rank;
      perm[pos] = (int)(br * M + tok);
      rowscale[pos] = top_val[i];
      pos4[tok * 4 + br * 2 + k] = pos;
    }
    __syncthreads();
  }
}

template <int G>
__device__ __forceinline__ void head_ln(f32x4& v, const float* w, const float* b, int dh, int gl) {
  const float mean = group_sum<G>(v[0] + v[1] + v[2] + v[3]) / dh;
  const f32x4 d = {v[0] - mean, v[1] - mean, v[2] - mean, v[3] - mean};
  const float rstd = rsqrtf(group_sum<G>(d[0] * d[0] + d[1] * d[1] + d[2] * d[2] + d[3] * d[3]) / dh + 1e-5f);
  const f32x4 ww = *(const f32x4*)(w + 4 * gl), bb = *(const f32x4*)(b + 4 * gl);
  v = (f32x4){d[0] * rstd * ww[0] + bb[0], d[1] * rstd * ww[1] + bb[1], d[2] * rstd * ww[2] + bb[2],
              d[3] * rstd * ww[3] + bb[3]};
}

template <int G>
__global__ __launch_bounds__(256) void head_norm_kernel(float* __restrict__ qkv, int64_t units, int H, int dh,
                                                        const float* w, const float* b) {
  const int gl = threadIdx.x % G;
  const int64_t gid = (blockIdx.x * (int64_t)blockDim.x + threadIdx.x) / G;
  const int64_t ng = (int64_t)gridDim.x * blockDim.x / G;
  for (int64_t u = gid; u < units; u += ng) {
    float* p = qkv + u * dh + 4 * gl;
    f32x4 v = *(const f32x4*)p;
    head_ln<G>(v, w, b, dh, gl);
    const int which = (int)((u / H) % 3);
    if (which < 2) {
      const float n = sqrtf(group_sum<G>(v[0] * v[0] + v[1] * v[1] + v[2] * v[2] + v[3] * v[3]));
      const float inv = 1.f / fmaxf(n, 1e-12f);
      v *= inv;
    }
    *(f32x4*)p = v;
  }
}

template <int G>
__global__ __launch_bounds__(256) void den_ln_kernel(const float* __restrict__ num, const float* __restrict__ phi,
                                                     int64_t M, int H, int dh, const float* w, const float* b,
                                                     void* __restrict__ out, int out_bf) {
  const int gl = threadIdx.x % G;
  const int64_t gid = (blockIdx.x * (int64_t)blockDim.x + threadIdx.x) / G;
  const int64_t ng = (int64_t)gridDim.x * blockDim.x / G;
  for (int64_t u = gid; u < M * H; u += ng) {
    const int64_t tok = u / H, h = u - tok * H;
    const f32x4 qf = *(const f32x4*)(phi + (tok * 2 * H + h) * dh + 4 * gl);
    const f32x4 kf = *(const f32x4*)(phi + (tok * 2 * H + H + h) * dh + 4 * gl);
    float den = group_sum<G>(qf[0] * kf[0] + qf[1] * kf[1] + qf[2] * kf[2] + qf[3] * kf[3]);
    den = fmaxf(den, 1e-6f);
    f32x4 v = *(const f32x4*)(num + u * dh + 4 * gl);
    v = (f32x4){v[0] / den, v[1] / den, v[2] / den, v[3] / den};
    head_ln<G>(v, w, b, dh, gl);
    if (out_bf) {
      *(uint2*)((uint16_t*)out + u * dh + 4 * gl) = make_uint2(pack_h16(out_bf, v[0], v[1]), pack_h16(out_bf, v[2], v[3]));
    } else {
      *(f32x4*)((float*)out + u * dh + 4 * gl) = v;
    }
  }
}

template <int G>
__global__ __launch_bounds__(256) void head_softmax_kernel(float* __restrict__ q, int64_t units, int dh) {
  const int gl = threadIdx.x % G;
  const int64_t gid = (blockIdx.x * (int64_t)blockDim.x + threadIdx.x) / G;
  const int64_t ng = (int64_t)gridDim.x * blockDim.x / G;
  for (int64_t u = gid; u < units; u += ng) {
    float* p = q + u * dh + 4 * gl;
    f32x4 v = *(const f32x4*)p;
    const float mx = group_max<G>(fmaxf(fmaxf(v[0], v[1]), fmaxf(v[2], v[3])));
    v = (f32x4){expf(v[0] - mx), expf(v[1] - mx), expf(v[2] - mx), expf(v[3] - mx)};
    const float s = group_sum<G>(v[0] + v[1] + v[2] + v[3]);
    *(f32x4*)p = (f32x4){v[0] / s, v[1] / s, v[2] / s, v[3] / s};
  }
}

#define MDM_HEAD_DISPATCH(dh, CALL)                 \
  do {                                              \
    switch (dh) {                                   \
      case 16: CALL(4); break;                      \
      case 32: CALL(8); break;                      \
      case 64: CALL(16); break;                     \
// ... 238 lines not shown
  if (g_variant == MDM_VAR_ROUTER_RUNTIME_E) return false;
  return g_variant == MDM_VAR_ROUTER_CONST_E || ((nv == 8 || nv == 16) && (E == 8 || E == 16));
}
template <int NV, int EX, int HNF, bool FAST = true>
bool launch_gate16_const(int grid, int smem, hipStream_t s, const float* x, int64_t M, int D, int E, const MoeGateParams& p) {
  static DevInt attr_done;
  if (smem > 65536 && smem > attr_done) {
    if (hipFuncSetAttribute((const void*)moe_gate16_kernel<NV, FAST, EX, HNF>, hipFuncAttributeMaxDynamicSharedMemorySize, smem) != hipSuccess)
      return false;
    attr_done = smem;
  }
  hipLaunchKernelGGL((moe_gate16_kernel<NV, FAST, EX, HNF>), dim3(grid), dim3(256), smem, s, x, M, D, E, p);
  return true;
}
template <int NV, int EX>
bool gate16_const_fmt(int grid, int smem, hipStream_t s, const float* x, int64_t M, int D, int E, const MoeGateParams& p) {
  switch (p.hn_bf16) {
    case 1: return launch_gate16_const<NV, EX, 1>(grid, smem, s, x, M, D, E, p);
    case 2: return launch_gate16_const<NV, EX, 2>(grid, smem, s, x, M, D, E, p);
    case 0:
      if constexpr (NV == 8 && EX == 8) return launch_gate16_const<NV, EX, 0, false>(grid, smem, s, x, M, D, E, p);
      return false;
    case 4:
      if constexpr (NV == 8 && EX == 8) return launch_gate16_const<NV, EX, 4, false>(grid, smem, s, x, M, D, E, p);
      return false;
    default: return false;
  }
}
bool gate16_const(int nv, int grid, int smem, hipStream_t s, const float* x, int64_t M, int D, int E, const MoeGateParams& p) {
  if (nv == 8 && E == 8) return gate16_const_fmt<8, 8>(grid, smem, s, x, M, D, E, p);
  if (nv == 8 && E == 16) return gate16_const_fmt<8, 16>(grid, smem, s, x, M, D, E, p);
  if (nv == 16 && E == 8) return gate16_const_fmt<16, 8>(grid, smem, s, x, M, D, E, p);
  if (nv == 16 && E == 16) return gate16_const_fmt<16, 16>(grid, smem, s, x, M, D, E, p);
  return false;
}

int moe_route(const float* x, int64_t M, int D, int E, const MoeGateParams& p, int* goff, int* cursor, int* perm,
              float* rowscale, int* pos4, hipStream_t s) {
  if (M <= 0) return MDM_OK;
  if (E < 2 || E > 16 || !x || !p.hn || !p.hist || !p.uimp || !p.top_idx || !p.top_val) return MDM_ERR_ARG;
  int nparts = 0;
  const int nv = D % 64 == 0 ? D / 64 : 0;
  if (nv == 1 || nv == 2 || nv == 4 || nv == 8 || nv == 16) {
    const int smem = 2 * E * D * 4 + 4 * D * 4 + 3 * 32 * 4;
    int64_t nb = (M + 15) / 16;
    const int grid = (int)(nb > 512 ? 512 : nb);
    nparts = grid;
    static DevInt attr_done;
    if (smem > 65536 && smem > attr_done) {
      const void* fns[4] = {(const void*)moe_gate16_kernel<16, true>, (const void*)moe_gate16_kernel<16, false>,
                            (const void*)moe_gate16_kernel<8, true>, (const void*)moe_gate16_kernel<8, false>};
      for (const void* fn : fns)
        if (hipFuncSetAttribute(fn, hipFuncAttributeMaxDynamicSharedMemorySize, smem) != hipSuccess) return MDM_ERR_LAUNCH;
      attr_done = smem;
    }
#define GATE16(NV)                                                                                            \
  do {                                                                                                        \
    if (gate16_const_wanted(NV, E) && gate16_const(NV, grid, smem, s, x, M, D, E, p)) {                      \
    } else if (p.hn_bf16 && p.hn_bf16 != 4) {                                                                 \
      hipLaunchKernelGGL((moe_gate16_kernel<NV, true>), dim3(grid), dim3(256), smem, s, x, M, D, E, p);       \
    } else {                                                                                                  \
      hipLaunchKernelGGL((moe_gate16_kernel<NV, false>), dim3(grid), dim3(256), smem, s, x, M, D, E, p);      \
    }                                                                                                         \
  } while (0)
    switch (D / 64) {
      case 1: GATE16(1); break;
      case 2: GATE16(2); break;
      case 4: GATE16(4); break;
      case 8: GATE16(8); break;
      case 16: GATE16(16); break;
      default: return MDM_ERR_UNSUPPORTED;
    }
#undef GATE16
  } else {
  const int gate_grid = row_grid(M) > 512 ? 512 : row_grid(M);
  nparts = gate_grid;
#define CALL(NE, VEC) hipLaunchKernelGGL((moe_gate_kernel<NE, VEC>), dim3(gate_grid), dim3(256), 0, s, x, M, D, E, p)
  MDM_ROW_DISPATCH(D, CALL);
#undef CALL
  }
  hipLaunchKernelGGL(moe_offsets_kernel, dim3(1), dim3(1024), 0, s, p.hist, p.uimp, nparts, E, goff, cursor, p);
  const int64_t total = 4 * M;
  int blocks = (int)((total + 255) / 256);
  hipLaunchKernelGGL(moe_assign_kernel, dim3(blocks > 1024 ? 1024 : blocks), dim3(256), 0, s, p.top_idx, p.top_val, M, E,
                     goff, cursor, perm, rowscale, pos4);
  MDM_RETURN_IF_LAUNCH_FAILED();
  return MDM_OK;
}

int head_norm(float* qkv, int64_t M, int H, int dh, const float* w, const float* b, hipStream_t s) {
  if (M <= 0) return MDM_OK;
  const int64_t units = M * 3 * H;
#define CALL(G) hipLaunchKernelGGL((head_norm_kernel<G>), dim3(unit_grid(units, G)), dim3(256), 0, s, qkv, units, H, dh, w, b)
  MDM_HEAD_DISPATCH(dh, CALL);
#undef CALL
  MDM_RETURN_IF_LAUNCH_FAILED();
  return MDM_OK;
}

int den_ln(const float* num, const float* phi, int64_t M, int H, int dh, const float* w, const float* b, void* out,
           int out_bf, hipStream_t s) {
  if (M <= 0) return MDM_OK;
#define CALL(G) \
  hipLaunchKernelGGL((den_ln_kernel<G>), dim3(unit_grid(M * H, G)), dim3(256), 0, s, num, phi, M, H, dh, w, b, out, out_bf)
  MDM_HEAD_DISPATCH(dh, CALL);
#undef CALL
  MDM_RETURN_IF_LAUNCH_FAILED();
  return MDM_OK;
}

int head_softmax(float* q, int64_t units, int dh, hipStream_t s) {
  if (units <= 0) return MDM_OK;
#define CALL(G) hipLaunchKernelGGL((head_softmax_kernel<G>), dim3(unit_grid(units, G)), dim3(256), 0, s, q, units, dh)
  MDM_HEAD_DISPATCH(dh, CALL);
#undef CALL
  MDM_RETURN_IF_LAUNCH_FAILED();
  return MDM_OK;
}

int row_softmax(float* sc, int64_t rows, int N, hipStream_t s, const int32_t* ntok, int64_t rows_per_b) {
  if (rows <= 0) return MDM_OK;
  if (N < 1 || N > 128 || rows_per_b < 1) return MDM_ERR_UNSUPPORTED;
  hipLaunchKernelGGL(row_softmax_kernel, dim3(unit_grid(rows, 32)), dim3(256), 0, s, sc, rows, N, ntok, rows_per_b);
  MDM_RETURN_IF_LAUNCH_FAILED();
  return MDM_OK;
}

int col_softmax(float* k, int B, int N, int D, hipStream_t s, const int32_t* ntok) {
  const int64_t n = (int64_t)B * D;
  if (n <= 0) return MDM_OK;
  hipLaunchKernelGGL(col_softmax_kernel, dim3((unsigned)((n + 255) / 256)), dim3(256), 0, s, k, B, N, D, ntok);
  MDM_RETURN_IF_LAUNCH_FAILED();
  return MDM_OK;
}

int sd_fold_mask_cb(float* cb, int B, int np, int hpp, int N, const int32_t* ntok, hipStream_t s) {
  const int n = B * np * 128;
  if (n <= 0 || !ntok) return MDM_OK;
  if (!cb || N < 1) return MDM_ERR_ARG;
  hipLaunchKernelGGL(sd_fold_mask_cb_kernel, dim3((n + 255) / 256), dim3(256), 0, s, cb, B, np, hpp, N, ntok);
  MDM_RETURN_IF_LAUNCH_FAILED();
  return MDM_OK;
}

int sinusoid(const int64_t* t, int B, int D, float* out, hipStream_t s) {
  hipLaunchKernelGGL(sinusoid_kernel, dim3((B * D + 255) / 256), dim3(256), 0, s, t, B, D, out);
  MDM_RETURN_IF_LAUNCH_FAILED();
  return MDM_OK;
}

int gated_mix(const float* t, const float* x, int64_t n, float* out, hipStream_t s) {
  hipLaunchKernelGGL(gated_mix_kernel, dim3((unsigned)((n + 255) / 256)), dim3(256), 0, s, t, x, n, out);
  MDM_RETURN_IF_LAUNCH_FAILED();
  return MDM_OK;
}

int text_assemble(const float* pp, const float* ph, int B, int N0, int P, int Dt, float* xf_out, float* xf_proj,
                  hipStream_t s) {
  hipLaunchKernelGGL(text_assemble_kernel, dim3((B * Dt + 255) / 256), dim3(256), 0, s, pp, ph, B, N0, P, Dt, xf_out, xf_proj);
  MDM_RETURN_IF_LAUNCH_FAILED();
  return MDM_OK;
}

int gated_mix_gather(const float* table, const int64_t* ts, int steps, const float* x, int B, int D, float* out,
                     uint16_t* out16, int h16, hipStream_t s) {
  hipLaunchKernelGGL(gated_mix_gather_kernel, dim3((B * D + 255) / 256), dim3(256), 0, s, table, ts, steps, x, B, D, out, out16, h16);
  MDM_RETURN_IF_LAUNCH_FAILED();
  return MDM_OK;
// ... 76 lines not shown
```

motiondiffusion-moe_amd/csrc/style_gemm.hip:

```cpp
#include "gemm.h"
#include "kernels.h"
#include "row.h"

namespace mdm {
namespace {

constexpr int SG_NT = 512, SG_D = 512, SG_NJ = 4;

__device__ __forceinline__ void sg_barrier() {
  asm volatile("s_waitcnt lgkmcnt(0)" ::: "memory");
  __builtin_amdgcn_s_barrier();
  asm volatile("" ::: "memory");
}

struct StyleGemmArgs {
  const void* src;
  int64_t M;
  int S;
  const float *pw, *pb;
  const float *sw, *sb;
  const float* sc;
  const int* pos4;
  const uint16_t* ws;
  const float* bias;
  const float* resid;
  float out_scale;
  const float* colscale;
  float* out;
  uint16_t* out16;
  const float *lw, *lb;
  float* ln_out;
  const float* skip;
  float skip_scale;
  const float *l2w, *l2b;
  int ln_x2;
};

template <typename HT, bool SRC16, int SG_RT>
__global__ __launch_bounds__(SG_NT, (SG_RT <= 2 ? 4 : 2)) void style_gemm_kernel(const StyleGemmArgs g) {
  constexpr int SG_ROWS = 16 * SG_RT, RPW = SG_ROWS / 8;
  typedef typename HT::frag_t frag_t;
  typedef Row<8, true> R8;
  constexpr int D = SG_D, FMT = HT::FMT;
  extern __shared__ __attribute__((aligned(1024))) uint8_t smem[];
  const int tid = threadIdx.x, lane = tid & 63;
  const int wn = __builtin_amdgcn_readfirstlane(tid >> 6);
  const int64_t row0 = (int64_t)blockIdx.x * SG_ROWS;

  const uint8_t* wp = (const uint8_t*)g.ws + (int64_t)wn * 64 * 1024 + lane * 16;
  constexpr int NR = SG_RT <= 2 ? 16 : 8;
  frag_t R[NR];
#pragma unroll
  for (int f = 0; f < 8; ++f) R[f] = *(const frag_t*)(wp + f * 1024);

  {
    R8 pww, pbb, sww, sbb;
    if (g.pw) pww.load(g.pw, D, lane), pbb.load(g.pb, D, lane);
    sww.load(g.sw, D, lane), sbb.load(g.sb, D, lane);
#pragma unroll 2
    for (int q = 0; q < RPW; ++q) {
      const int rl = RPW * wn + q;
      int64_t row = row0 + rl;
      row = row < g.M ? row : g.M - 1;
      const float* scb = g.sc + (row / g.S) * 2 * (int64_t)D;
      R8 r, scale, shift;
      scale.load(scb, D, lane);
      shift.load(scb + D, D, lane);
      if (g.pos4) {
        const int p0 = g.pos4[row * 4 + 0], p1 = g.pos4[row * 4 + 1], p2 = g.pos4[row * 4 + 2], p3 = g.pos4[row * 4 + 3];
        R8 a, b, c, d;
        if constexpr (SRC16) {
          const uint16_t* xh = (const uint16_t*)g.src;
          a.template load_h16<FMT>(xh + (int64_t)p0 * D, D, lane);
          b.template load_h16<FMT>(xh + (int64_t)p1 * D, D, lane);
          c.template load_h16<FMT>(xh + (int64_t)p2 * D, D, lane);
          d.template load_h16<FMT>(xh + (int64_t)p3 * D, D, lane);
        } else {
          const float* x = (const float*)g.src;
          a.load(x + (int64_t)p0 * D, D, lane);
          b.load(x + (int64_t)p1 * D, D, lane);
          c.load(x + (int64_t)p2 * D, D, lane);
          d.load(x + (int64_t)p3 * D, D, lane);
        }
#pragma unroll
        for (int j = 0; j < 8; ++j) r.e[j] = ((a.e[j] + b.e[j]) + (c.e[j] + d.e[j])) * 0.5f;
      } else {
        if constexpr (SRC16) {
          r.template load_h16<FMT>((const uint16_t*)g.src + row * D, D, lane);
        } else {
          r.load((const float*)g.src + row * D, D, lane);
        }
      }
      if (g.pw) {
        r.layernorm(pww, pbb, D, lane);
        float s = 0.f;
#pragma unroll
        for (int j = 0; j < 8; ++j) s += r.e[j] * r.e[j];
        const float inv = sqrtf((float)D) / fmaxf(sqrtf(wave_sum(s)), 1e-12f);
#pragma unroll
        for (int j = 0; j < 8; ++j) r.e[j] *= inv;
      }
      r.layernorm(sww, sbb, D, lane);
#pragma unroll
      for (int j = 0; j < 8; ++j) r.e[j] = silu(r.e[j] * (1.f + scale.e[j]) + shift.e[j]);
      uint8_t* ir = smem + rl * 1024 + (lane & 1) * 8;
      *(uint2*)(ir + ((((lane >> 1)) ^ (rl & 15)) << 4)) = make_uint2(HT::pack(r.e[0], r.e[1]), HT::pack(r.e[2], r.e[3]));
      *(uint2*)(ir + (((32 + (lane >> 1)) ^ (rl & 15)) << 4)) = make_uint2(HT::pack(r.e[4], r.e[5]), HT::pack(r.e[6], r.e[7]));
    }
  }
#pragma unroll
  for (int f = 8; f < NR; ++f) R[f] = *(const frag_t*)(wp + f * 1024);
  wp += NR * 1024;
  sg_barrier();

  const int frow = lane & 15, fq = lane >> 4;
  f32x4 y[SG_RT][SG_NJ];
#pragma unroll
  for (int i = 0; i < SG_RT; ++i)
#pragma unroll
    for (int j = 0; j < SG_NJ; ++j) y[i][j] = (f32x4){0.f, 0.f, 0.f, 0.f};
  {
    const int xb = frow * 1024 + ((fq ^ frow) << 4);
    frag_t A[2][SG_RT];
#pragma unroll
    for (int i = 0; i < SG_RT; ++i) A[0][i] = *(const frag_t*)(smem + xb + i * 16384);
#pragma unroll
    for (int s = 0; s < 16; ++s) {
      if (s + 1 < 16) {
#pragma unroll
        for (int i = 0; i < SG_RT; ++i) A[(s + 1) & 1][i] = *(const frag_t*)(smem + (xb ^ (64 * ((s + 1) & 3))) + ((s + 1) >> 2) * 256 + i * 16384);
      }
#pragma unroll
      for (int j = 0; j < SG_NJ; ++j) {
        const int slot = (s * SG_NJ + j) & (NR - 1);
#pragma unroll
        for (int i = 0; i < SG_RT; ++i) y[i][j] = HT::mfma16(R[slot], A[s & 1][i], y[i][j]);
        R[slot] = *(const frag_t*)(wp + slot * 1024);
        if (slot == NR - 1) wp += NR * 1024;
      }
      __builtin_amdgcn_sched_barrier(0);
    }
  }

  sg_barrier();
  float* stg = (float*)smem;
#pragma unroll
  for (int j = 0; j < SG_NJ; ++j) {
    const int n = wn * 64 + 16 * j + 4 * fq;
    f32x4 bb = *(const f32x4*)(g.bias + n);
    f32x4 cs = {g.out_scale, g.out_scale, g.out_scale, g.out_scale};
    if (g.colscale) {
      const f32x4 q = *(const f32x4*)(g.colscale + n);
      cs[0] *= q[0], cs[1] *= q[1], cs[2] *= q[2], cs[3] *= q[3];
    }
#pragma unroll
    for (int i = 0; i < SG_RT; ++i) {
      const int ml = i * 16 + frow;
      f32x4 v = y[i][j];
      v[0] = (v[0] + bb[0]) * cs[0], v[1] = (v[1] + bb[1]) * cs[1], v[2] = (v[2] + bb[2]) * cs[2], v[3] = (v[3] + bb[3]) * cs[3];
      *(f32x4*)(stg + ml * D + (((n >> 2) ^ (ml & 31)) << 2)) = v;
    }
  }
  const int cl = tid & 127, n = 4 * cl;
  f32x4 q[SG_ROWS / 4];
#pragma unroll
  for (int k = 0; k < SG_ROWS / 4; ++k) {
    int64_t m = row0 + (tid >> 7) + 4 * k;
    m = m < g.M ? m : g.M - 1;
    q[k] = g.resid ? *(const f32x4*)(g.resid + m * D + n) : (f32x4){0.f, 0.f, 0.f, 0.f};
  }
  sg_barrier();
#pragma unroll
  for (int k = 0; k < SG_ROWS / 4; ++k) {
    const int ml = (tid >> 7) + 4 * k;
    const int64_t m = row0 + ml;
    if (m >= g.M) continue;
    f32x4 v = *(const f32x4*)(stg + ml * D + ((cl ^ (ml & 31)) << 2));
    if (g.resid) v[0] += q[k][0], v[1] += q[k][1], v[2] += q[k][2], v[3] += q[k][3];
    *(f32x4*)(g.out + m * D + n) = v;
    if (g.out16) *(uint2*)(g.out16 + m * D + n) = make_uint2(HT::pack(v[0], v[1]), HT::pack(v[2], v[3]));
  }
}

template <int SG_RT>
__global__ __launch_bounds__(SG_NT, (SG_RT <= 2 ? 4 : 2)) void style_gemm3_kernel(const StyleGemmArgs g) {
  constexpr int SG_ROWS = 16 * SG_RT, RPW = SG_ROWS / 8;
  typedef HB::frag_t frag_t;
  typedef Row<8, true> R8;
  constexpr int D = SG_D, IMG = SG_ROWS * 1024;
  extern __shared__ __attribute__((aligned(1024))) uint8_t smem[];
  uint8_t* const imh = smem;
  uint8_t* const iml = smem + IMG;
  const int tid = threadIdx.x, lane = tid & 63;
  const int wn = __builtin_amdgcn_readfirstlane(tid >> 6);
  const int64_t row0 = (int64_t)blockIdx.x * SG_ROWS;

  const uint8_t* wp = (const uint8_t*)g.ws + (int64_t)wn * 128 * 1024 + lane * 16;
  constexpr int NR = SG_RT <= 2 ? 8 : 16;
  frag_t R[NR];
#pragma unroll
  for (int f = 0; f < (NR < 8 ? NR : 8); ++f) R[f] = *(const frag_t*)(wp + f * 1024);

  {
    R8 pww, pbb, sww, sbb;
    if (g.pw) pww.load(g.pw, D, lane), pbb.load(g.pb, D, lane);
    sww.load(g.sw, D, lane), sbb.load(g.sb, D, lane);
#pragma unroll 2
    for (int q = 0; q < RPW; ++q) {
      const int rl = RPW * wn + q;
      int64_t row = row0 + rl;
      row = row < g.M ? row : g.M - 1;
      const float* scb = g.sc + (row / g.S) * 2 * (int64_t)D;
      R8 r, scale, shift;
      scale.load(scb, D, lane);
      shift.load(scb + D, D, lane);
      const float* x = (const float*)g.src;
      if (g.pos4) {
        const int p0 = g.pos4[row * 4 + 0], p1 = g.pos4[row * 4 + 1], p2 = g.pos4[row * 4 + 2], p3 = g.pos4[row * 4 + 3];
        R8 a, b, c, d;
        a.load(x + (int64_t)p0 * D, D, lane);
        b.load(x + (int64_t)p1 * D, D, lane);
        c.load(x + (int64_t)p2 * D, D, lane);
        d.load(x + (int64_t)p3 * D, D, lane);
#pragma unroll
        for (int j = 0; j < 8; ++j) r.e[j] = ((a.e[j] + b.e[j]) + (c.e[j] + d.e[j])) * 0.5f;
      } else {
        r.load(x + row * D, D, lane);
      }
      if (g.pw) {
        r.layernorm(pww, pbb, D, lane);
        float s = 0.f;
#pragma unroll
        for (int j = 0; j < 8; ++j) s += r.e[j] * r.e[j];
        const float inv = sqrtf((float)D) / fmaxf(sqrtf(wave_sum(s)), 1e-12f);
#pragma unroll
        for (int j = 0; j < 8; ++j) r.e[j] *= inv;
      }
      r.layernorm(sww, sbb, D, lane);
#pragma unroll
      for (int j = 0; j < 8; ++j) r.e[j] = silu(r.e[j] * (1.f + scale.e[j]) + shift.e[j]);
      uint32_t h0, h1, h2, h3, l0, l1, l2, l3;
      split_bf16(r.e[0], r.e[1], h0, l0);
      split_bf16(r.e[2], r.e[3], h1, l1);
      split_bf16(r.e[4], r.e[5], h2, l2);
      split_bf16(r.e[6], r.e[7], h3, l3);
      const int o0 = rl * 1024 + ((((lane >> 1)) ^ (rl & 15)) << 4) + (lane & 1) * 8;
      const int o1 = rl * 1024 + (((32 + (lane >> 1)) ^ (rl & 15)) << 4) + (lane & 1) * 8;
      *(uint2*)(imh + o0) = make_uint2(h0, h1), *(uint2*)(imh + o1) = make_uint2(h2, h3);
      *(uint2*)(iml + o0) = make_uint2(l0, l1), *(uint2*)(iml + o1) = make_uint2(l2, l3);
    }
  }
#pragma unroll
  for (int f = 8; f < NR; ++f) R[f] = *(const frag_t*)(wp + f * 1024);
  wp += NR * 1024;
  sg_barrier();

  const int frow = lane & 15, fq = lane >> 4;
  f32x4 y[SG_RT][SG_NJ];
#pragma unroll
  for (int i = 0; i < SG_RT; ++i)
#pragma unroll
    for (int j = 0; j < SG_NJ; ++j) y[i][j] = (f32x4){0.f, 0.f, 0.f, 0.f};
  {
// ... 58 lines not shown
    }
    R8 lww, lbb, l2ww, l2bb;
    if (g.lw) lww.load(g.lw, D, lane), lbb.load(g.lb, D, lane);
    if (g.l2w) l2ww.load(g.l2w, D, lane), l2bb.load(g.l2b, D, lane);
#pragma unroll
    for (int q = 0; q < RPW; ++q) {
      const int rl = RPW * wn + q;
      const int64_t m = row0 + rl;
      if (m >= g.M) continue;
      const f32x4 v0 = *(const f32x4*)(stg + rl * D + ((lane ^ (rl & 31)) << 2));
      const f32x4 v1 = *(const f32x4*)(stg + rl * D + (((64 + lane) ^ (rl & 31)) << 2));
      R8 r;
      r.e[0] = v0[0], r.e[1] = v0[1], r.e[2] = v0[2], r.e[3] = v0[3], r.e[4] = v1[0], r.e[5] = v1[1], r.e[6] = v1[2], r.e[7] = v1[3];
      if (g.resid) {
#pragma unroll
        for (int j = 0; j < 8; ++j) r.e[j] += xr[q].e[j];
      }
      if (g.skip) {
#pragma unroll
        for (int j = 0; j < 8; ++j) r.e[j] = sk[q].e[j] + g.skip_scale * r.e[j];
        r.layernorm(lww, lbb, D, lane);
        r.store(g.out + m * D, D, lane);
        if (g.l2w) {
          r.layernorm(l2ww, l2bb, D, lane);
          if (g.ln_x2) r.store_x2((uint16_t*)g.ln_out + m * 2 * D, D, lane);
          else r.store(g.ln_out + m * D, D, lane);
        }
      } else {
        r.store(g.out + m * D, D, lane);
        if (g.lw) {
          r.layernorm(lww, lbb, D, lane);
          if (g.ln_x2) r.store_x2((uint16_t*)g.ln_out + m * 2 * D, D, lane);
          else r.store(g.ln_out + m * D, D, lane);
        }
      }
    }
  }
}

__global__ __launch_bounds__(256) void gemm_stream3_pack_kernel(const float* w, uint16_t* out) {
  for (int fi = blockIdx.x * 4 + (threadIdx.x >> 6); fi < 8 * 64; fi += gridDim.x * 4) {
    const int l = threadIdx.x & 63, wv = fi >> 6, f = fi & 63, s = f >> 2, j = f & 3;
    const float* src = w + (int64_t)(64 * wv + 16 * j + (l & 15)) * SG_D + 32 * s + 8 * (l >> 4);
    uint4 h, lo;
    split_bf16(src[0], src[1], h.x, lo.x);
    split_bf16(src[2], src[3], h.y, lo.y);
    split_bf16(src[4], src[5], h.z, lo.z);
    split_bf16(src[6], src[7], h.w, lo.w);
    *(uint4*)(out + (int64_t)fi * 1024 + l * 8) = h;
    *(uint4*)(out + (int64_t)fi * 1024 + 512 + l * 8) = lo;
  }
}

template <typename HT>
__global__ __launch_bounds__(256) void gemm_stream_pack_kernel(const float* w, uint16_t* out) {
  for (int fi = blockIdx.x * 4 + (threadIdx.x >> 6); fi < 8 * 64; fi += gridDim.x * 4) {
    const int l = threadIdx.x & 63, wv = fi >> 6, f = fi & 63, s = f >> 2, j = f & 3;
    const float* src = w + (int64_t)(64 * wv + 16 * j + (l & 15)) * SG_D + 32 * s + 8 * (l >> 4);
    uint4 o;
    o.x = HT::pack(src[0], src[1]), o.y = HT::pack(src[2], src[3]), o.z = HT::pack(src[4], src[5]), o.w = HT::pack(src[6], src[7]);
    *(uint4*)(out + (int64_t)fi * 512 + l * 8) = o;
  }
}

}

int64_t gemm_stream_elems(int N, int K) { return (N == SG_D && K == SG_D) ? (int64_t)N * K + 16 * 512 : 0; }

int gemm_stream_pack(const float* w, int N, int K, int h16, uint16_t* out, hipStream_t stream) {
  if (!w || !out || N != SG_D || K != SG_D) return MDM_ERR_UNSUPPORTED;
  if (hipMemsetAsync(out + (int64_t)N * K, 0, 16 * 512 * sizeof(uint16_t), stream) != hipSuccess) return MDM_ERR_LAUNCH;
  if (h16 == MDM_H16_F16) {
    hipLaunchKernelGGL(gemm_stream_pack_kernel<HF>, dim3(128), dim3(256), 0, stream, w, out);
  } else {
    hipLaunchKernelGGL(gemm_stream_pack_kernel<HB>, dim3(128), dim3(256), 0, stream, w, out);
  }
  MDM_RETURN_IF_LAUNCH_FAILED();
  return MDM_OK;
}

bool style_gemm_supported(int D, int64_t M) { return D == SG_D && M > 0 && M / 32 < (1ll << 30); }


template <int RT>
static int launch_style_gemm(const StyleGemmArgs& g, bool src16, int h16, hipStream_t s) {
  constexpr int smem = 16 * RT * SG_D * 4;
  static DevOnce attr;
  if (!attr) {
    const void* fns[4] = {(const void*)style_gemm_kernel<HB, true, RT>, (const void*)style_gemm_kernel<HB, false, RT>,
                          (const void*)style_gemm_kernel<HF, true, RT>, (const void*)style_gemm_kernel<HF, false, RT>};
    for (const void* fn : fns)
      if (hipFuncSetAttribute(fn, hipFuncAttributeMaxDynamicSharedMemorySize, smem) != hipSuccess) return MDM_ERR_LAUNCH;
    attr = true;
  }
  const dim3 grid((unsigned)((g.M + 16 * RT - 1) / (16 * RT)));
  if (h16 == MDM_H16_F16) {
    if (src16) hipLaunchKernelGGL((style_gemm_kernel<HF, true, RT>), grid, dim3(SG_NT), smem, s, g);
    else hipLaunchKernelGGL((style_gemm_kernel<HF, false, RT>), grid, dim3(SG_NT), smem, s, g);
  } else {
    if (src16) hipLaunchKernelGGL((style_gemm_kernel<HB, true, RT>), grid, dim3(SG_NT), smem, s, g);
    else hipLaunchKernelGGL((style_gemm_kernel<HB, false, RT>), grid, dim3(SG_NT), smem, s, g);
  }
  MDM_RETURN_IF_LAUNCH_FAILED();
  return MDM_OK;
}

int style_gemm(const void* src, int src_fmt, int64_t M, int D, int S, const float* pw, const float* pb, const float* sw, const float* sb,
               const float* sc, const int* pos4, const uint16_t* ws, const float* bias, const float* resid, float out_scale,
               const float* colscale, float* out, uint16_t* out16, int h16, hipStream_t s) {
  if (M <= 0) return MDM_OK;
  if (!style_gemm_supported(D, M)) return MDM_ERR_UNSUPPORTED;
  if (!src || !sw || !sb || !sc || !ws || !bias || !out || S <= 0 || (pw && !pb)) return MDM_ERR_ARG;
  if ((h16 != MDM_H16_BF16 && h16 != MDM_H16_F16) || (src_fmt != 0 && src_fmt != h16) || ((uintptr_t)ws & 15)) return MDM_ERR_ARG;
  StyleGemmArgs g = {};
  g.src = src, g.M = M, g.S = S, g.pw = pw, g.pb = pb, g.sw = sw, g.sb = sb, g.sc = sc, g.pos4 = pos4, g.ws = ws, g.bias = bias;
  g.resid = resid, g.out_scale = out_scale, g.colscale = colscale, g.out = out, g.out16 = out16;
  return launch_style_gemm<2>(g, src_fmt != 0, h16, s);
}

int64_t gemm_stream3_elems(int N, int K) { return (N == SG_D && K == SG_D) ? 2 * (int64_t)N * K + 16 * 512 : 0; }

int gemm_stream3_pack(const float* w, int N, int K, uint16_t* out, hipStream_t stream) {
  if (!w || !out || N != SG_D || K != SG_D) return MDM_ERR_UNSUPPORTED;
  if (hipMemsetAsync(out + 2 * (int64_t)N * K, 0, 16 * 512 * sizeof(uint16_t), stream) != hipSuccess) return MDM_ERR_LAUNCH;
  hipLaunchKernelGGL(gemm_stream3_pack_kernel, dim3(128), dim3(256), 0, stream, w, out);
  MDM_RETURN_IF_LAUNCH_FAILED();
  return MDM_OK;
}

template <int RT>
static int launch_style_gemm3(const StyleGemmArgs& g, hipStream_t s) {
  constexpr int smem = 16 * RT * SG_D * 4;
  static DevOnce attr;
  if (!attr) {
    if (hipFuncSetAttribute((const void*)style_gemm3_kernel<RT>, hipFuncAttributeMaxDynamicSharedMemorySize, smem) != hipSuccess) return MDM_ERR_LAUNCH;
    attr = true;
  }
  const dim3 grid((unsigned)((g.M + 16 * RT - 1) / (16 * RT)));
  hipLaunchKernelGGL((style_gemm3_kernel<RT>), grid, dim3(SG_NT), smem, s, g);
  MDM_RETURN_IF_LAUNCH_FAILED();
  return MDM_OK;
}

int style_gemm3(const float* src, int64_t M, int D, int S, const float* pw, const float* pb, const float* sw, const float* sb,
                const float* sc, const int* pos4, const uint16_t* ws3, const float* bias, const float* resid, float out_scale,
                const float* colscale, float* out, const StyleTail3& t, hipStream_t s) {
  if (M <= 0) return MDM_OK;
  if (!style_gemm_supported(D, M)) return MDM_ERR_UNSUPPORTED;
  if (!src || !sw || !sb || !sc || !ws3 || !bias || !out || S <= 0 || (pw && !pb) || ((uintptr_t)ws3 & 15)) return MDM_ERR_ARG;
  if ((t.lw && !t.lb) || (t.skip && (!t.lw || !t.lb)) || (t.l2w && (!t.l2b || !t.skip)) || ((t.skip ? t.l2w != nullptr : t.lw != nullptr) != (t.ln_out != nullptr)))
    return MDM_ERR_ARG;
  StyleGemmArgs g = {};
  g.src = src, g.M = M, g.S = S, g.pw = pw, g.pb = pb, g.sw = sw, g.sb = sb, g.sc = sc, g.pos4 = pos4, g.ws = ws3, g.bias = bias;
  g.resid = resid, g.out_scale = out_scale, g.colscale = colscale, g.out = out;
  g.lw = t.lw, g.lb = t.lb, g.ln_out = t.ln_out, g.skip = t.skip, g.skip_scale = t.skip_scale, g.l2w = t.l2w, g.l2b = t.l2b, g.ln_x2 = t.ln_x2;
  return launch_style_gemm3<2>(g, s);
}

}
```

Baseline: 239.8 denoising-steps/sec.

## Fold MoE gate LayerNorm and routing logits into cross-attention style GEMM epilogue

The cross-attention stylization GEMM epilogue now stages its output tile in LDS, loads the gate weights and LayerNorm parameters, and computes the MoE gate LayerNorm, normalized hidden writes, top-k logits and per-block histograms for each row. A lighter assign kernel (moe_route_folded) then consumes those partial results, so the separate routing kernel no longer has to re-read the block output. The goal is to cut one kernel launch and a full pass over the activations per layer, at the price of more LDS and registers in the style GEMM, which could lower its occupancy. The old path is still reachable through a variant flag.

```diff
diff --git a/include/mdm_hip.h b/include/mdm_hip.h
--- a/include/mdm_hip.h
+++ b/include/mdm_hip.h
@@ -372,10 +372,12 @@
   MDM_VAR_STREAM3_NEVER = 69,
   MDM_VAR_STREAM3_ALWAYS = 70
 };
+enum MdmRouteVariant { MDM_VAR_ROUTE_LAUNCH = 171 };
 int mdm_set_gemm_variant(int variant);
 
 int mdm_probe_enable(int32_t enable);
 int mdm_route_dump(int32_t* buf, int64_t capacity);
+int mdm_route_workspace(const MdmModel* m, int32_t B, int32_t T, int32_t N, int64_t* off);
 int mdm_sd_fold_passes(int32_t D, int32_t H, int32_t N);
 int mdm_probe_read(float* us, int32_t* rows, int32_t cap);
 
diff --git a/motiondiffusion-moe_amd/_lib.py b/motiondiffusion-moe_amd/_lib.py
--- a/motiondiffusion-moe_amd/_lib.py
+++ b/motiondiffusion-moe_amd/_lib.py
@@ -152,7 +152,7 @@
 EXPORTS = ["mdm_version", "mdm_gemm", "mdm_fused_mlp", "mdm_mlp_stream_elems", "mdm_mlp_stream_pack", "mdm_gemm_stream_elems", "mdm_gemm_stream_pack", "mdm_gemm_stream3_elems", "mdm_gemm_stream3_pack", "mdm_gemm_stream1_elems", "mdm_gemm_stream1_pack", "mdm_gemm_stream3x_elems", "mdm_gemm_stream3x_group_elems", "mdm_gemm_stream3x_pack", "mdm_pack_bf16", "mdm_pack_f16", "mdm_pack_fp8", "mdm_workspace_bytes", "mdm_text_cache_build",
            "mdm_denoiser_forward", "mdm_stem_cache_build", "mdm_block_forward", "mdm_moe_ffn_forward", "mdm_dual_self_attn_forward", "mdm_linear_xattn_forward",
            "mdm_softmax_xattn_ffn_forward", "mdm_performer_attn_forward", "mdm_stylization_forward", "mdm_stem_embeddings",
-           "mdm_cfg_posterior_step", "mdm_ddim_step", "mdm_fill_timesteps_mapped", "mdm_guided_update", "mdm_guided_update_inpaint", "mdm_composed_update", "mdm_noise_normal", "mdm_noise_normal_ids", "mdm_text_head_workspace_bytes", "mdm_text_head_forward", "mdm_motion_postprocess", "mdm_motion_features_max_frames", "mdm_motion_features", "mdm_motion_fk_max_frames", "mdm_motion_fk", "mdm_foot_skate_max_frames", "mdm_foot_skate", "mdm_joint_control_max_frames", "mdm_joint_loss_grad", "mdm_joint_guidance", "mdm_handshake_blend", "mdm_xattn_gate", "mdm_fill_i64", "mdm_add_i32", "mdm_set_gemm_variant", "mdm_probe_enable", "mdm_probe_read", "mdm_route_dump",
+           "mdm_cfg_posterior_step", "mdm_ddim_step", "mdm_fill_timesteps_mapped", "mdm_guided_update", "mdm_guided_update_inpaint", "mdm_composed_update", "mdm_noise_normal", "mdm_noise_normal_ids", "mdm_text_head_workspace_bytes", "mdm_text_head_forward", "mdm_motion_postprocess", "mdm_motion_features_max_frames", "mdm_motion_features", "mdm_motion_fk_max_frames", "mdm_motion_fk", "mdm_foot_skate_max_frames", "mdm_foot_skate", "mdm_joint_control_max_frames", "mdm_joint_loss_grad", "mdm_joint_guidance", "mdm_handshake_blend", "mdm_xattn_gate", "mdm_fill_i64", "mdm_add_i32", "mdm_set_gemm_variant", "mdm_probe_enable", "mdm_probe_read", "mdm_route_dump", "mdm_route_workspace",
            "mdm_moe_train_workspace_bytes", "mdm_moe_ffn_train_forward", "mdm_moe_ffn_train_backward", "mdm_sumsq", "mdm_adam_step", "mdm_sd_fold_passes",
            "mdm_gru_bidir_workspace_bytes", "mdm_gru_bidir", "mdm_eval_pad_rows", "mdm_eval_ln_leaky", "mdm_eval_matching", "mdm_eval_center"]
 
diff --git a/motiondiffusion-moe_amd/csrc/api.hip b/motiondiffusion-moe_amd/csrc/api.hip
--- a/motiondiffusion-moe_amd/csrc/api.hip
+++ b/motiondiffusion-moe_amd/csrc/api.hip
@@ -63,6 +63,7 @@
     case MDM_VAR_STREAM_ALWAYS:
     case MDM_VAR_STREAM3_NEVER:
     case MDM_VAR_STREAM3_ALWAYS:
+    case MDM_VAR_ROUTE_LAUNCH:
       mdm::g_variant = v;
       return MDM_OK;
     default:
diff --git a/motiondiffusion-moe_amd/csrc/gemm.h b/motiondiffusion-moe_amd/csrc/gemm.h
--- a/motiondiffusion-moe_amd/csrc/gemm.h
+++ b/motiondiffusion-moe_amd/csrc/gemm.h
@@ -102,11 +102,19 @@
   const float *l2w = nullptr, *l2b = nullptr;
   int ln_x2 = 0;
 };
+struct MoeGateParams;
+struct StyleRoute {
+  const MoeGateParams* gate = nullptr;
+  int E = 0;
+  int* cursor = nullptr;
+};
+bool style_gemm_route_supported(int D, int64_t M, int E, int hn_fmt, int h16);
+int64_t style_gemm_route_parts(int64_t M);
 int style_gemm3(const float* src, int64_t M, int D, int S, const float* pw, const float* pb, const float* sw, const float* sb,
                 const float* sc, const int* pos4, const uint16_t* ws3, const float* bias, const float* resid, float out_scale,
                 const float* colscale, float* out, const StyleTail3& t, hipStream_t s);
 int style_gemm(const void* src, int src_fmt, int64_t M, int D, int S, const float* pw, const float* pb, const float* sw, const float* sb,
                const float* sc, const int* pos4, const uint16_t* ws, const float* bias, const float* resid, float out_scale,
-               const float* colscale, float* out, uint16_t* out16, int h16, hipStream_t s);
+               const float* colscale, float* out, uint16_t* out16, int h16, hipStream_t s, const StyleRoute* route = nullptr);
 
 }
diff --git a/motiondiffusion-moe_amd/csrc/kernels.h b/motiondiffusion-moe_amd/csrc/kernels.h
--- a/motiondiffusion-moe_amd/csrc/kernels.h
+++ b/motiondiffusion-moe_amd/csrc/kernels.h
@@ -31,6 +31,8 @@
 int f16_to_bf16x2(const uint16_t* src, int64_t n, uint16_t* hi, uint16_t* lo, hipStream_t s);
 int moe_route(const float* x, int64_t M, int D, int E, const MoeGateParams& p, int* goff, int* cursor, int* perm,
               float* rowscale, int* pos4, hipStream_t s);
+int moe_route_folded(int64_t M, int E, const MoeGateParams& p, int nparts, int* goff, int* cursor, int* perm, float* rowscale,
+                     int* pos4, hipStream_t s);
 int head_norm(float* qkv, int64_t M, int H, int dh, const float* w, const float* b, hipStream_t s);
 int den_ln(const float* num, const float* phi, int64_t M, int H, int dh, const float* w, const float* b, void* out,
            int out_bf, hipStream_t s);
diff --git a/motiondiffusion-moe_amd/csrc/model.hip b/motiondiffusion-moe_amd/csrc/model.hip
--- a/motiondiffusion-moe_amd/csrc/model.hip
+++ b/motiondiffusion-moe_amd/csrc/model.hip
@@ -221,13 +221,14 @@
 
 int style_apply(const Ctx& c, const MdmStyle& st, const float* src, const float* pw, const float* pb, const int* pos4,
                 const float* sc, float* tmp, const float* resid, float out_scale, const float* colscale, float* out,
-                uint16_t* out16 = nullptr, bool src_bf16 = false, const StyleTail3* t3 = nullptr) {
+                uint16_t* out16 = nullptr, bool src_bf16 = false, const StyleTail3* t3 = nullptr, const StyleRoute* route = nullptr) {
   const int D = c.m->D;
   const StylePath path = style_path(c, st, src_bf16, out16 != nullptr, t3 != nullptr);
+  if (route && path != StylePath::FUSED16) return MDM_ERR_UNSUPPORTED;
   switch (path) {
     case StylePath::FUSED16:
       return style_gemm(src, src_bf16 ? c.h16 : 0, c.M, D, c.S, pw, pb, st.norm_w, st.norm_b, sc, pos4, st.out_ws, st.out_b, resid,
-                        out_scale, colscale, out, out16, c.h16, c.s);
+                        out_scale, colscale, out, out16, c.h16, c.s, route);
     case StylePath::FUSED3:
     case StylePath::FUSED3_TAIL:
       return style_gemm3(src, c.M, D, c.S, pw, pb, st.norm_w, st.norm_b, sc, pos4, st.out_ws3, st.out_b, resid, out_scale, colscale, out,
@@ -427,8 +428,28 @@
   return XattnPath::CHAIN;
 }
 
+enum class RoutePath { FOLDED, LAUNCH };
+RoutePath route_path(const Ctx& c, const MdmLayer& l) {
+  if (g_variant == MDM_VAR_ROUTE_LAUNCH || g_variant == MDM_VAR_ROUTER_CONST_E || g_variant == MDM_VAR_ROUTER_RUNTIME_E) return RoutePath::LAUNCH;
+  if (c.bf && !c.fp8 && style_path(c, l.ca_style, true, false, false) == StylePath::FUSED16 &&
+      style_gemm_route_supported(c.m->D, c.M, c.m->E, fmt_mlp(c), c.h16))
+    return RoutePath::FOLDED;
+  return RoutePath::LAUNCH;
+}
+MoeGateParams gate_params(const Ctx& c, const MdmLayer& l, const int* forced) {
+  const Work& w = c.w;
+  MoeGateParams p = {};
+  for (int b = 0; b < 2; ++b) {
+    p.ln_w[b] = l.moe_ln_w[b], p.ln_b[b] = l.moe_ln_b[b];
+    p.gate_w[b] = l.gate_w[b], p.gate_b[b] = l.gate_b[b];
+    p.usage[b] = l.usage[b], p.importance[b] = l.importance[b];
+  }
+  p.hn = w.hn, p.hn_bf16 = c.fp8 ? 3 : fmt_mlp(c), p.hn_scale = w.hn_scale, p.top_idx = w.top_idx, p.top_val = w.top_val, p.hist = w.hist, p.uimp = w.uimp, p.forced_idx = forced;
+  return p;
+}
+
 int cross_block(const Ctx& c, const MdmLayer& l, const float* at, const float* x, const float* sc, float* out,
-                bool pre_normed = false) {
+                bool pre_normed = false, const StyleRoute* route = nullptr) {
   const MdmModel& m = *c.m;
   const int D = m.D, H = m.H, dh = D / H;
   const Work& w = c.w;
@@ -464,7 +485,7 @@
       break;
     }
   }
-  return style_apply(c, l.ca_style, w.t4, nullptr, nullptr, nullptr, sc, w.t2, x, 1.f, l.ca_gvec, out, nullptr, y16);
+  return style_apply(c, l.ca_style, w.t4, nullptr, nullptr, nullptr, sc, w.t2, x, 1.f, l.ca_gvec, out, nullptr, y16, nullptr, route);
 }
 
 GemmArgs expert_gemm(const Ctx& c, const void* A, int K, const MdmPacked& W, const float* bias, int N) {
@@ -495,18 +516,17 @@
 }
 
 int moe_block(const Ctx& c, const MdmLayer& l, const float* x, const float* sc, const int* forced, float* out,
-              uint16_t* out16, int32_t* route_out = nullptr) {
+              uint16_t* out16, int32_t* route_out = nullptr, RoutePath rp = RoutePath::LAUNCH) {
   const MdmModel& m = *c.m;
   const int D = m.D, F = m.F, E = m.E;
   const Work& w = c.w;
-  MoeGateParams p = {};
-  for (int b = 0; b < 2; ++b) {
-    p.ln_w[b] = l.moe_ln_w[b], p.ln_b[b] = l.moe_ln_b[b];
-    p.gate_w[b] = l.gate_w[b], p.gate_b[b] = l.gate_b[b];
-    p.usage[b] = l.usage[b], p.importance[b] = l.importance[b];
-  }
-  p.hn = w.hn, p.hn_bf16 = c.fp8 ? 3 : fmt_mlp(c), p.hn_scale = w.hn_scale, p.top_idx = w.top_idx, p.top_val = w.top_val, p.hist = w.hist, p.uimp = w.uimp, p.forced_idx = forced;
-  MDM_TRY(moe_route(x, c.M, D, E, p, w.goff, w.cursor, w.perm, w.rowscale, w.pos4, c.s));
+  const MoeGateParams p = gate_params(c, l, forced);
+  switch (rp) {
+    case RoutePath::FOLDED:
+      MDM_TRY(moe_route_folded(c.M, E, p, (int)style_gemm_route_parts(c.M), w.goff, w.cursor, w.perm, w.rowscale, w.pos4, c.s));
+      break;
+    case RoutePath::LAUNCH: MDM_TRY(moe_route(x, c.M, D, E, p, w.goff, w.cursor, w.perm, w.rowscale, w.pos4, c.s)); break;
+  }
   if (route_out && hipMemcpyAsync(route_out, w.top_idx, 4 * c.M * sizeof(int32_t), hipMemcpyDeviceToDevice, c.s) != hipSuccess)
     return MDM_ERR_LAUNCH;
   MdmMlpDesc f = {};
@@ -679,9 +699,13 @@
   if (!c.bf) x16 = y16 = nullptr;
   MDM_TRY(dual_block(c, l, x, x16, sc4, y, l.ca_norm_w, l.ca_norm_b));
   MDM_TRY(dump(0, y));
-  MDM_TRY(cross_block(c, l, tc_at(m, tc, layer), y, sc4 + 2 * scs, x, true));
+  const RoutePath rp = route_path(c, l);
+  const MoeGateParams gp = gate_params(c, l, forced);
+  StyleRoute sr;
+  sr.gate = &gp, sr.E = m.E, sr.cursor = c.w.cursor;
+  MDM_TRY(cross_block(c, l, tc_at(m, tc, layer), y, sc4 + 2 * scs, x, true, rp == RoutePath::FOLDED ? &sr : nullptr));
   MDM_TRY(dump(1, x));
-  MDM_TRY(moe_block(c, l, x, sc4 + 3 * scs, forced, y, y16, route_out));
+  MDM_TRY(moe_block(c, l, x, sc4 + 3 * scs, forced, y, y16, route_out, rp));
   MDM_TRY(dump(2, y));
   MDM_TRY(sdcross_block(c, l, tc_k(m, tc, layer), tc_v(m, tc, layer), y, y16, x, x16, tc_fold(m, tc, layer)));
   return dump(3, x);
@@ -1087,6 +1111,15 @@
 
 int mdm_sd_fold_passes(int32_t D, int32_t H, int32_t N) { return sd_fold_policy(D, H, N); }
 
+int mdm_route_workspace(const MdmModel* m, int32_t B, int32_t T, int32_t N, int64_t* off) {
+  if (check_model(m) != MDM_OK || B <= 0 || T <= 0 || !off) return MDM_ERR_ARG;
+  uint8_t* const base = (uint8_t*)4096;
+  const Work w = carve(*m, B, T, N, base);
+  const void* p[8] = {w.hn, w.top_idx, w.top_val, w.perm, w.rowscale, w.pos4, w.goff, w.cursor};
+  for (int i = 0; i < 8; ++i) off[i] = (const uint8_t*)p[i] - base;
+  return MDM_OK;
+}
+
 int mdm_route_dump(int32_t* buf, int64_t capacity) {
   if (buf && capacity <= 0) return MDM_ERR_ARG;
   g_route_dump = buf, g_route_cap = buf ? capacity : 0;
diff --git a/motiondiffusion-moe_amd/csrc/moe_gate_row.h b/motiondiffusion-moe_amd/csrc/moe_gate_row.h
--- /dev/null
+++ b/motiondiffusion-moe_amd/csrc/moe_gate_row.h
@@ -0,0 +1,141 @@
+#pragma once
+#include "kernels.h"
+#include "mdm_common.h"
+
+namespace mdm {
+namespace {
+
+__host__ __device__ constexpr int gate16_lds_bytes(int E, int D) { return 2 * E * D * 4 + 4 * D * 4 + 3 * 32 * 4; }
+
+template <int NV>
+__device__ __forceinline__ float gate16_row_sum(const f32x4 (&v)[NV]) {
+  float s = 0.f;
+#pragma unroll
+  for (int c = 0; c < NV; ++c) s += v[c][0] + v[c][1] + v[c][2] + v[c][3];
+  return s;
+}
+
+template <int NV, bool FAST, int EX, int HNF, int EB = 16>
+__device__ __forceinline__ void gate16_row(f32x4 (&v)[NV], float s, int64_t row, bool ok, int64_t rc, int64_t M, int E, int hnf, int l16,
+                                           const float* gw, const float* lnw, const float* lnb, int* s_hist, float* s_usage,
+                                           float* s_imp, const MoeGateParams& p) {
+  constexpr int D = 64 * NV;
+  const float mean = group_sum<16>(s) / D;
+  float q = 0.f;
+#pragma unroll
+  for (int c = 0; c < NV; ++c) {
+    v[c] = (f32x4){v[c][0] - mean, v[c][1] - mean, v[c][2] - mean, v[c][3] - mean};
+    q += v[c][0] * v[c][0] + v[c][1] * v[c][1] + v[c][2] * v[c][2] + v[c][3] * v[c][3];
+  }
+  const float rstd = rsqrtf(group_sum<16>(q) / D + 1e-5f);
+#pragma unroll
+  for (int br = 0; br < 2; ++br) {
+    float logit[16];
+#pragma unroll
+    for (int e = 0; e < 16; ++e) logit[e] = 0.f;
+    float amax = 0.f;
+#pragma unroll
+    for (int c = 0; c < NV; ++c) {
+      const int k = 4 * (l16 + 16 * c);
+      const f32x4 w = *(const f32x4*)(lnw + br * D + k), b = *(const f32x4*)(lnb + br * D + k);
+      const f32x4 h = {v[c][0] * rstd * w[0] + b[0], v[c][1] * rstd * w[1] + b[1], v[c][2] * rstd * w[2] + b[2],
+                       v[c][3] * rstd * w[3] + b[3]};
+      amax = fmaxf(amax, fmaxf(fmaxf(fabsf(h[0]), fabsf(h[1])), fmaxf(fabsf(h[2]), fabsf(h[3]))));
+      if constexpr (HNF >= 0) {
+        if constexpr (HNF == 1 || HNF == 2) {
+          *(uint2*)((uint16_t*)p.hn + ((int64_t)br * M + rc) * D + k) = make_uint2(pack_h16(HNF, h[0], h[1]), pack_h16(HNF, h[2], h[3]));
+        } else if constexpr (HNF == 0) {
+          *(f32x4*)((float*)p.hn + ((int64_t)br * M + rc) * D + k) = h;
+        } else if constexpr (HNF == 4) {
+          static_assert(D % 32 == 0, "lane pairs of store_x2_4p hold k and k ^ 4 of one 32-column block");
+          store_x2_4p((uint16_t*)p.hn + ((int64_t)br * M + rc) * 2 * D, k, h[0], h[1], h[2], h[3]);
+        }
+      } else if (ok && p.hn_bf16 != 3) {
+        if (p.hn_bf16 == 4) {
+          store_x2_4((uint16_t*)p.hn + ((int64_t)br * M + row) * 2 * D, k, h[0], h[1], h[2], h[3]);
+        } else if (p.hn_bf16 == 2) {
+          *(uint2*)((uint16_t*)p.hn + ((int64_t)br * M + row) * D + k) = make_uint2(pack_h16(2, h[0], h[1]), pack_h16(2, h[2], h[3]));
+        } else if (p.hn_bf16) {
+          *(uint2*)((uint16_t*)p.hn + ((int64_t)br * M + row) * D + k) = make_uint2(pack_h16(1, h[0], h[1]), pack_h16(1, h[2], h[3]));
+        } else {
+          *(f32x4*)((float*)p.hn + ((int64_t)br * M + row) * D + k) = h;
+        }
+      }
+#pragma unroll
+      for (int e = 0; e < 16; ++e)
+        if (e < E) {
+          const f32x4 g = *(const f32x4*)(gw + (br * E + e) * D + k);
+          if constexpr (FAST) {
+            logit[e] = __builtin_fmaf(h[3], g[3], __builtin_fmaf(h[2], g[2], __builtin_fmaf(h[1], g[1], __builtin_fmaf(h[0], g[0], logit[e]))));
+          } else {
+            logit[e] += h[0] * g[0] + h[1] * g[1] + h[2] * g[2] + h[3] * g[3];
+          }
+          if constexpr (EX > 0 && HNF >= 0 && EB < 16)
+            if ((e + 1) % EB == 0 && e + 1 < EX) __builtin_amdgcn_sched_barrier(0);
+        }
+      if constexpr (EX > 0 && HNF >= 0) __builtin_amdgcn_sched_barrier(0);
+    }
+    if (hnf == 3) {
+      amax = group_max<16>(amax);
+      const float scale = amax > 0.f ? amax * (1.f / 448.f) : 1.f, inv = 1.f / scale;
+#pragma unroll
+      for (int c = 0; c < NV; ++c) {
+        const int k = 4 * (l16 + 16 * c);
+        const f32x4 w = *(const f32x4*)(lnw + br * D + k), b = *(const f32x4*)(lnb + br * D + k);
+        uint32_t q8 = 0;
+        q8 = __builtin_amdgcn_cvt_pk_fp8_f32((v[c][0] * rstd * w[0] + b[0]) * inv, (v[c][1] * rstd * w[1] + b[1]) * inv, q8, false);
+        q8 = __builtin_amdgcn_cvt_pk_fp8_f32((v[c][2] * rstd * w[2] + b[2]) * inv, (v[c][3] * rstd * w[3] + b[3]) * inv, q8, true);
+        if (HNF >= 0 || ok) *(uint32_t*)((uint8_t*)p.hn + ((int64_t)br * M + (HNF >= 0 ? rc : row)) * D + k) = q8;
+      }
+      if (ok && l16 == 0) p.hn_scale[(int64_t)br * M + row] = scale;
+    }
+    float mx = -INFINITY, mine = -INFINITY;
+#pragma unroll
+    for (int e = 0; e < 16; ++e) {
+      if (e < E) {
+        logit[e] = group_sum<16>(logit[e]) + p.gate_b[br][e];
+        mx = fmaxf(mx, logit[e]);
+        mine = (l16 == e) ? logit[e] : mine;
+      }
+    }
+    const float den = group_sum<16>(l16 < E ? expf(mine - mx) : 0.f);
+    int i1 = 0, i2 = 1;
+    float l1 = -INFINITY, l2 = -INFINITY;
+    if (p.forced_idx) {
+      i1 = min(max(p.forced_idx[((int64_t)br * M + rc) * 2 + 0], 0), E - 1);
+      i2 = min(max(p.forced_idx[((int64_t)br * M + rc) * 2 + 1], 0), E - 1);
+#pragma unroll
+      for (int e = 0; e < 16; ++e) {
+        l1 = e == i1 ? logit[e] : l1;
+        l2 = e == i2 ? logit[e] : l2;
+      }
+    } else {
+#pragma unroll
+      for (int e = 0; e < 16; ++e) {
+        if (e < E) {
+          if (logit[e] > l1) {
+            l2 = l1, i2 = i1;
+            l1 = logit[e], i1 = e;
+          } else if (logit[e] > l2) {
+            l2 = logit[e], i2 = e;
+          }
+        }
+      }
+      if (i2 == i1) i2 = i1 == 0 ? 1 : 0;
+    }
+    const float v1 = expf(l1 - mx) / den, v2 = expf(l2 - mx) / den;
+    if (ok && l16 == 0) {
+      const int64_t o = ((int64_t)br * M + row) * 2;
+      p.top_idx[o] = i1, p.top_idx[o + 1] = i2;
+      p.top_val[o] = v1, p.top_val[o + 1] = v2;
+      atomicAdd(&s_hist[br * E + i1], 1);
+      atomicAdd(&s_hist[br * E + i2], 1);
+      atomicAdd(&s_usage[br * E + i1], 1.f);
+      atomicAdd(&s_imp[br * E + i1], v1);
+      atomicAdd(&s_imp[br * E + i2], v2);
+    }
+  }
+}
+
+}
+}
diff --git a/motiondiffusion-moe_amd/csrc/rowwise.hip b/motiondiffusion-moe_amd/csrc/rowwise.hip
--- a/motiondiffusion-moe_amd/csrc/rowwise.hip
+++ b/motiondiffusion-moe_amd/csrc/rowwise.hip
@@ -1,4 +1,5 @@
 #include "kernels.h"
+#include "moe_gate_row.h"
 #include "row.h"
 
 namespace mdm {
@@ -257,127 +258,12 @@
     const int64_t rc = ok ? row : M - 1;
     if constexpr (NV > 8) load_x(base, vn);
     f32x4 v[NV];
-    float s = 0.f;
-#pragma unroll
-    for (int c = 0; c < NV; ++c) {
-      v[c] = vn[c];
-      s += v[c][0] + v[c][1] + v[c][2] + v[c][3];
-    }
+#pragma unroll
+    for (int c = 0; c < NV; ++c) v[c] = vn[c];
+    const float s = gate16_row_sum(v);
     if constexpr (NV <= 8)
       if (base + stride < M) load_x(base + stride, vn);
-    const float mean = group_sum<16>(s) / D;
-    float q = 0.f;
-#pragma unroll
-    for (int c = 0; c < NV; ++c) {
-      v[c] = (f32x4){v[c][0] - mean, v[c][1] - mean, v[c][2] - mean, v[c][3] - mean};
-      q += v[c][0] * v[c][0] + v[c][1] * v[c][1] + v[c][2] * v[c][2] + v[c][3] * v[c][3];
-    }
-    const float rstd = rsqrtf(group_sum<16>(q) / D + 1e-5f);
-#pragma unroll
-    for (int br = 0; br < 2; ++br) {
-      float logit[16];
-#pragma unroll
-      for (int e = 0; e < 16; ++e) logit[e] = 0.f;
-      float amax = 0.f;
-#pragma unroll
-      for (int c = 0; c < NV; ++c) {
-        const int k = 4 * (l16 + 16 * c);
-        const f32x4 w = *(const f32x4*)(lnw + br * D + k), b = *(const f32x4*)(lnb + br * D + k);
-        const f32x4 h = {v[c][0] * rstd * w[0] + b[0], v[c][1] * rstd * w[1] + b[1], v[c][2] * rstd * w[2] + b[2],
-                         v[c][3] * rstd * w[3] + b[3]};
-        amax = fmaxf(amax, fmaxf(fmaxf(fabsf(h[0]), fabsf(h[1])), fmaxf(fabsf(h[2]), fabsf(h[3]))));
-        if constexpr (HNF >= 0) {
-          if constexpr (HNF == 1 || HNF == 2) {
-            *(uint2*)((uint16_t*)p.hn + ((int64_t)br * M + rc) * D + k) = make_uint2(pack_h16(HNF, h[0], h[1]), pack_h16(HNF, h[2], h[3]));
-          } else if constexpr (HNF == 0) {
-            *(f32x4*)((float*)p.hn + ((int64_t)br * M + rc) * D + k) = h;
-          } else if constexpr (HNF == 4) {
-            static_assert(D % 32 == 0, "lane pairs of store_x2_4p hold k and k ^ 4 of one 32-column block");
-            store_x2_4p((uint16_t*)p.hn + ((int64_t)br * M + rc) * 2 * D, k, h[0], h[1], h[2], h[3]);
-          }
-        } else if (ok && p.hn_bf16 != 3) {
-          if (p.hn_bf16 == 4) {
-            store_x2_4((uint16_t*)p.hn + ((int64_t)br * M + row) * 2 * D, k, h[0], h[1], h[2], h[3]);
-          } else if (p.hn_bf16 == 2) {
-            *(uint2*)((uint16_t*)p.hn + ((int64_t)br * M + row) * D + k) = make_uint2(pack_h16(2, h[0], h[1]), pack_h16(2, h[2], h[3]));
-          } else if (p.hn_bf16) {
-            *(uint2*)((uint16_t*)p.hn + ((int64_t)br * M + row) * D + k) = make_uint2(pack_h16(1, h[0], h[1]), pack_h16(1, h[2], h[3]));
-          } else {
-            *(f32x4*)((float*)p.hn + ((int64_t)br * M + row) * D + k) = h;
-          }
-        }
-#pragma unroll
-        for (int e = 0; e < 16; ++e)
-          if (e < E) {
-            const f32x4 g = *(const f32x4*)(gw + (br * E + e) * D + k);
-            if constexpr (FAST) {
-              logit[e] = __builtin_fmaf(h[3], g[3], __builtin_fmaf(h[2], g[2], __builtin_fmaf(h[1], g[1], __builtin_fmaf(h[0], g[0], logit[e]))));
-            } else {
-              logit[e] += h[0] * g[0] + h[1] * g[1] + h[2] * g[2] + h[3] * g[3];
-            }
-          }
-        if constexpr (EX > 0 && HNF >= 0) __builtin_amdgcn_sched_barrier(0);
-      }
-      if (hnf == 3) {
-        amax = group_max<16>(amax);
-        const float scale = amax > 0.f ? amax * (1.f / 448.f) : 1.f, inv = 1.f / scale;
-#pragma unroll
-        for (int c = 0; c < NV; ++c) {
-          const int k = 4 * (l16 + 16 * c);
-          const f32x4 w = *(const f32x4*)(lnw + br * D + k), b = *(const f32x4*)(lnb + br * D + k);
-          uint32_t q = 0;
-          q = __builtin_amdgcn_cvt_pk_fp8_f32((v[c][0] * rstd * w[0] + b[0]) * inv, (v[c][1] * rstd * w[1] + b[1]) * inv, q, false);
-          q = __builtin_amdgcn_cvt_pk_fp8_f32((v[c][2] * rstd * w[2] + b[2]) * inv, (v[c][3] * rstd * w[3] + b[3]) * inv, q, true);
-          if (HNF >= 0 || ok) *(uint32_t*)((uint8_t*)p.hn + ((int64_t)br * M + (HNF >= 0 ? rc : row)) * D + k) = q;
-        }
-        if (ok && l16 == 0) p.hn_scale[(int64_t)br * M + row] = scale;
-      }
-      float mx = -INFINITY, mine = -INFINITY;
-#pragma unroll
-      for (int e = 0; e < 16; ++e) {
-        if (e < E) {
-          logit[e] = group_sum<16>(logit[e]) + p.gate_b[br][e];
-          mx = fmaxf(mx, logit[e]);
-          mine = (l16 == e) ? logit[e] : mine;
-        }
-      }
-      const float den = group_sum<16>(l16 < E ? expf(mine - mx) : 0.f);
-      int i1 = 0, i2 = 1;
-      float l1 = -INFINITY, l2 = -INFINITY;
-      if (p.forced_idx) {
-        i1 = min(max(p.forced_idx[((int64_t)br * M + rc) * 2 + 0], 0), E - 1);
-        i2 = min(max(p.forced_idx[((int64_t)br * M + rc) * 2 + 1], 0), E - 1);
-#pragma unroll
-        for (int e = 0; e < 16; ++e) {
-          l1 = e == i1 ? logit[e] : l1;
-          l2 = e == i2 ? logit[e] : l2;
-        }
-      } else {
-#pragma unroll
-        for (int e = 0; e < 16; ++e) {
-          if (e < E) {
-            if (logit[e] > l1) {
-              l2 = l1, i2 = i1;
-              l1 = logit[e], i1 = e;
-            } else if (logit[e] > l2) {
-              l2 = logit[e], i2 = e;
-            }
-          }
-        }
-        if (i2 == i1) i2 = i1 == 0 ? 1 : 0;
-      }
-      const float v1 = expf(l1 - mx) / den, v2 = expf(l2 - mx) / den;
-      if (ok && l16 == 0) {
-        const int64_t o = ((int64_t)br * M + row) * 2;
-        p.top_idx[o] = i1, p.top_idx[o + 1] = i2;
-        p.top_val[o] = v1, p.top_val[o + 1] = v2;
-        atomicAdd(&s_hist[br * E + i1], 1);
-        atomicAdd(&s_hist[br * E + i2], 1);
-        atomicAdd(&s_usage[br * E + i1], 1.f);
-        atomicAdd(&s_imp[br * E + i1], v1);
-        atomicAdd(&s_imp[br * E + i2], v2);
-      }
-    }
+    gate16_row<NV, FAST, EX, HNF>(v, s, row, ok, rc, M, E, hnf, l16, gw, lnw, lnb, s_hist, s_usage, s_imp, p);
   }
   __syncthreads();
   if (threadIdx.x < 2 * E) {
@@ -431,13 +317,92 @@
   }
 }
 
+template <bool OFFS>
 __global__ __launch_bounds__(256) void moe_assign_kernel(const int* __restrict__ top_idx, const float* __restrict__ top_val,
-                                                         int64_t M, int E, const int* __restrict__ goff,
+                                                         int64_t M, int E, int* __restrict__ goff,
                                                          int* __restrict__ cursor, int* __restrict__ perm,
-                                                         float* __restrict__ rowscale, int* __restrict__ pos4) {
-  __shared__ int s_cnt[32], s_base[32];
+                                                         float* __restrict__ rowscale, int* __restrict__ pos4, int nparts,
+                                                         MoeGateParams p) {
+  __shared__ int s_cnt[32], s_base[32], s_goff[33];
+  if constexpr (OFFS) {
+    __shared__ int tile[256][33];
+    __shared__ int chunk[8][33];
+    const int g = threadIdx.x & 31, c = threadIdx.x >> 5, G = 2 * E;
+    const bool book = blockIdx.x == gridDim.x - 1;
+    auto col_sums = [&](auto zero, const decltype(zero)* __restrict__ part, int ld) {
+      typedef decltype(zero) T;
+      T acc[32];
+#pragma unroll
+      for (int j = 0; j < 32; ++j) acc[j] = zero;
+      for (int b0 = threadIdx.x; b0 < nparts; b0 += 512) {
+        const int b1 = b0 + 256;
+        uint4 r0[8], r1[8];
+#pragma unroll
+        for (int j = 0; j < 8; ++j) r0[j] = 4 * j < G ? *(const uint4*)(part + (int64_t)b0 * ld + 4 * j) : make_uint4(0, 0, 0, 0);
+#pragma unroll
+        for (int j = 0; j < 8; ++j) r1[j] = 4 * j < G && b1 < nparts ? *(const uint4*)(part + (int64_t)b1 * ld + 4 * j) : make_uint4(0, 0, 0, 0);
+#pragma unroll
+        for (int j = 0; j < 8; ++j) {
+          const uint32_t w0[4] = {r0[j].x, r0[j].y, r0[j].z, r0[j].w}, w1[4] = {r1[j].x, r1[j].y, r1[j].z, r1[j].w};
+#pragma unroll
+          for (int i = 0; i < 4; ++i) {
+            acc[4 * j + i] += __builtin_bit_cast(T, w0[i]);
+            acc[4 * j + i] += __builtin_bit_cast(T, w1[i]);
+          }
+        }
+      }
+      __syncthreads();
+#pragma unroll
+      for (int j = 0; j < 32; ++j) tile[threadIdx.x][j] = __builtin_bit_cast(int, acc[j]);
+      __syncthreads();
+      T s = zero;
+      for (int i = 0; i < 32; ++i) s += __builtin_bit_cast(T, tile[32 * c + i][g]);
+      chunk[c][g] = __builtin_bit_cast(int, s);
+      __syncthreads();
+      if (threadIdx.x < 32) {
+        T t = zero;
+        for (int k = 0; k < 8; ++k) t += __builtin_bit_cast(T, chunk[k][g]);
+        chunk[0][g] = __builtin_bit_cast(int, t);
+      }
+      __syncthreads();
+    };
+    col_sums(0, p.hist, 32);
+    if (threadIdx.x < 32) s_cnt[g] = g < G ? chunk[0][g] : 0;
+    if (book) {
+      float ut = 0.f, it = 0.f;
+      col_sums(0.f, p.uimp, 64);
+      if (threadIdx.x < G) ut = __int_as_float(chunk[0][g]);
+      col_sums(0.f, p.uimp + 32, 64);
+      if (threadIdx.x < G) {
+        it = __int_as_float(chunk[0][g]);
+        const int br = g / E, e = g - br * E;
+        if (p.usage[br]) {
+          atomicAdd(&p.usage[br][e], ut);
+          atomicAdd(&p.importance[br][e], it);
+        }
+      }
+    }
+    __syncthreads();
+    if (threadIdx.x == 0) {
+      int s = 0;
+      for (int i = 0; i < G; ++i) {
+        s_goff[i] = s;
+        s += s_cnt[i];
+      }
+      s_goff[G] = s;
+    }
+    __syncthreads();
+    if (book) {
+      if (threadIdx.x <= G) goff[threadIdx.x] = s_goff[threadIdx.x];
+      return;
+    }
+  } else {
+    if (threadIdx.x <= 2 * E) s_goff[threadIdx.x] = goff[threadIdx.x];
+    __syncthreads();
+  }
   const int64_t total = 2 * M * 2;
-  for (int64_t base = blockIdx.x * (int64_t)blockDim.x; base < total; base += (int64_t)gridDim.x * blockDim.x) {
+  const int64_t nwork = OFFS ? gridDim.x - 1 : gridDim.x;
+  for (int64_t base = blockIdx.x * (int64_t)blockDim.x; base < total; base += nwork * blockDim.x) {
     if (threadIdx.x < 32) s_cnt[threadIdx.x] = 0;
     __syncthreads();
     const int64_t i = base + threadIdx.x;
@@ -455,7 +420,7 @@
     if (threadIdx.x < 2 * E && s_cnt[threadIdx.x]) s_base[threadIdx.x] = atomicAdd(&cursor[threadIdx.x], s_cnt[threadIdx.x]);
     __syncthreads();
     if (g >= 0) {
-      const int pos = goff[g] + s_base[g] + rank;
+      const int pos = s_goff[g] + s_base[g] + rank;
       perm[pos] = (int)(br * M + tok);
       rowscale[pos] = top_val[i];
       pos4[tok * 4 + br * 2 + k] = pos;
@@ -860,8 +825,20 @@
   hipLaunchKernelGGL(moe_offsets_kernel, dim3(1), dim3(1024), 0, s, p.hist, p.uimp, nparts, E, goff, cursor, p);
   const int64_t total = 4 * M;
   int blocks = (int)((total + 255) / 256);
-  hipLaunchKernelGGL(moe_assign_kernel, dim3(blocks > 1024 ? 1024 : blocks), dim3(256), 0, s, p.top_idx, p.top_val, M, E,
-                     goff, cursor, perm, rowscale, pos4);
+  hipLaunchKernelGGL(moe_assign_kernel<false>, dim3(blocks > 1024 ? 1024 : blocks), dim3(256), 0, s, p.top_idx, p.top_val, M, E,
+                     goff, cursor, perm, rowscale, pos4, nparts, p);
+  MDM_RETURN_IF_LAUNCH_FAILED();
+  return MDM_OK;
+}
+
+int moe_route_folded(int64_t M, int E, const MoeGateParams& p, int nparts, int* goff, int* cursor, int* perm, float* rowscale,
+                     int* pos4, hipStream_t s) {
+  if (M <= 0) return MDM_OK;
+  if (E < 2 || E > 16 || nparts < 1 || nparts > 1024 || !p.hist || !p.uimp || !p.top_idx || !p.top_val) return MDM_ERR_ARG;
+  const int64_t total = 4 * M;
+  int blocks = (int)((total + 255) / 256);
+  hipLaunchKernelGGL(moe_assign_kernel<true>, dim3((blocks > 1024 ? 1024 : blocks) + 1), dim3(256), 0, s, p.top_idx, p.top_val, M, E,
+                     goff, cursor, perm, rowscale, pos4, nparts, p);
   MDM_RETURN_IF_LAUNCH_FAILED();
   return MDM_OK;
 }
diff --git a/motiondiffusion-moe_amd/csrc/style_gemm.hip b/motiondiffusion-moe_amd/csrc/style_gemm.hip
--- a/motiondiffusion-moe_amd/csrc/style_gemm.hip
+++ b/motiondiffusion-moe_amd/csrc/style_gemm.hip
@@ -1,5 +1,6 @@
 #include "gemm.h"
 #include "kernels.h"
+#include "moe_gate_row.h"
 #include "row.h"
 
 namespace mdm {
@@ -36,8 +37,17 @@
   int ln_x2;
 };
 
-template <typename HT, bool SRC16, int SG_RT>
-__global__ __launch_bounds__(SG_NT, (SG_RT <= 2 ? 4 : 2)) void style_gemm_kernel(const StyleGemmArgs g) {
+struct StyleRouteArgs {
+  MoeGateParams p;
+  int* cursor;
+};
+
+constexpr int sg_lds_bytes(int RT, int RE) {
+  return RE > 0 && gate16_lds_bytes(RE, SG_D) > 16 * RT * SG_D * 4 ? gate16_lds_bytes(RE, SG_D) : 16 * RT * SG_D * 4;
+}
+
+template <typename HT, bool SRC16, int SG_RT, int RE = 0>
+__global__ __launch_bounds__(SG_NT, (SG_RT <= 2 ? 4 : 2)) void style_gemm_kernel(const StyleGemmArgs g, const StyleRouteArgs rt) {
   constexpr int SG_ROWS = 16 * SG_RT, RPW = SG_ROWS / 8;
   typedef typename HT::frag_t frag_t;
   typedef Row<8, true> R8;
@@ -179,6 +189,57 @@
     if (g.resid) v[0] += q[k][0], v[1] += q[k][1], v[2] += q[k][2], v[3] += q[k][3];
     *(f32x4*)(g.out + m * D + n) = v;
     if (g.out16) *(uint2*)(g.out16 + m * D + n) = make_uint2(HT::pack(v[0], v[1]), HT::pack(v[2], v[3]));
+    if constexpr (RE > 0) *(f32x4*)(stg + ml * D + ((cl ^ (ml & 31)) << 2)) = v;
+  }
+
+  if constexpr (RE > 0) {
+    static_assert(SG_ROWS * 16 == SG_NT, "one 16-lane group per row of the tile");
+    static_assert(2 * RE * D / 4 % (2 * SG_NT) == 0 && 4 * D / 4 == SG_NT, "staging loops below");
+    static_assert(sg_lds_bytes(SG_RT, RE) <= 80 * 1024, "two workgroups per CU");
+    constexpr int NV = D / 64, NG = 2 * RE * D / 4 / SG_NT;
+    const MoeGateParams& p = rt.p;
+    const int tid = wn * 64 + (int)__builtin_amdgcn_mbcnt_hi(~0u, __builtin_amdgcn_mbcnt_lo(~0u, 0u));
+    constexpr int NP = NG <= 4 ? NG : NG / 2;
+    f32x4 tg[NP];
+#pragma unroll
+    for (int j = 0; j < NP; ++j) tg[j] = *(const f32x4*)(p.gate_w[j / (NG / 2)] + 4 * (tid + SG_NT * (j % (NG / 2))));
+    const int lw = tid >> 7;
+    const f32x4 tl = *(const f32x4*)((lw < 2 ? p.ln_w[lw] : p.ln_b[lw - 2]) + 4 * (tid & 127));
+    sg_barrier();
+    const int l16 = tid & 15;
+    const int64_t row = row0 + (tid >> 4);
+    const bool ok = row < g.M;
+    const int64_t rc = ok ? row : g.M - 1;
+    const int rl = (int)(rc - row0);
+    f32x4 v[NV];
+#pragma unroll
+    for (int c = 0; c < NV; ++c) v[c] = *(const f32x4*)(stg + rl * D + (((l16 + 16 * c) ^ (rl & 31)) << 2));
+    sg_barrier();
+    float* gw = (float*)smem;
+    float* lnw = gw + 2 * RE * D;
+    float* lnb = lnw + 2 * D;
+    int* s_hist = (int*)(lnb + 2 * D);
+    float* s_usage = (float*)(s_hist + 32);
+    float* s_imp = s_usage + 32;
+#pragma unroll
+    for (int j = 0; j < NP; ++j) *(f32x4*)(gw + (j / (NG / 2)) * RE * D + 4 * (tid + SG_NT * (j % (NG / 2)))) = tg[j];
+    if constexpr (NP < NG) {
+#pragma unroll
+      for (int j = NP; j < NG; ++j) tg[j - NP] = *(const f32x4*)(p.gate_w[j / (NG / 2)] + 4 * (tid + SG_NT * (j % (NG / 2))));
+#pragma unroll
+      for (int j = NP; j < NG; ++j) *(f32x4*)(gw + (j / (NG / 2)) * RE * D + 4 * (tid + SG_NT * (j % (NG / 2)))) = tg[j - NP];
+    }
+    *(f32x4*)(lnw + 4 * tid) = tl;
+    if (tid < 32) s_hist[tid] = 0, s_usage[tid] = 0.f, s_imp[tid] = 0.f;
+    if (blockIdx.x == 0 && tid < 2 * RE) rt.cursor[tid] = 0;
+    sg_barrier();
+    gate16_row<NV, true, RE, FMT, (RE > 8 ? 4 : 16)>(v, gate16_row_sum(v), row, ok, rc, g.M, RE, FMT, l16, gw, lnw, lnb, s_hist, s_usage, s_imp, p);
+    __syncthreads();
+    if (tid < 2 * RE) {
+      p.hist[blockIdx.x * 32 + tid] = s_hist[tid];
+      p.uimp[blockIdx.x * 64 + tid] = s_usage[tid];
+      p.uimp[blockIdx.x * 64 + 32 + tid] = s_imp[tid];
+    }
   }
 }
 
@@ -403,32 +464,38 @@
 bool style_gemm_supported(int D, int64_t M) { return D == SG_D && M > 0 && M / 32 < (1ll << 30); }
 
 
-template <int RT>
-static int launch_style_gemm(const StyleGemmArgs& g, bool src16, int h16, hipStream_t s) {
-  constexpr int smem = 16 * RT * SG_D * 4;
+template <int RT, int RE = 0>
+static int launch_style_gemm(const StyleGemmArgs& g, const StyleRouteArgs& rt, bool src16, int h16, hipStream_t s) {
+  constexpr int smem = sg_lds_bytes(RT, RE);
   static DevOnce attr;
   if (!attr) {
-    const void* fns[4] = {(const void*)style_gemm_kernel<HB, true, RT>, (const void*)style_gemm_kernel<HB, false, RT>,
-                          (const void*)style_gemm_kernel<HF, true, RT>, (const void*)style_gemm_kernel<HF, false, RT>};
+    const void* fns[4] = {(const void*)style_gemm_kernel<HB, true, RT, RE>, (const void*)style_gemm_kernel<HB, false, RT, RE>,
+                          (const void*)style_gemm_kernel<HF, true, RT, RE>, (const void*)style_gemm_kernel<HF, false, RT, RE>};
     for (const void* fn : fns)
       if (hipFuncSetAttribute(fn, hipFuncAttributeMaxDynamicSharedMemorySize, smem) != hipSuccess) return MDM_ERR_LAUNCH;
     attr = true;
   }
   const dim3 grid((unsigned)((g.M + 16 * RT - 1) / (16 * RT)));
   if (h16 == MDM_H16_F16) {
-    if (src16) hipLaunchKernelGGL((style_gemm_kernel<HF, true, RT>), grid, dim3(SG_NT), smem, s, g);
-    else hipLaunchKernelGGL((style_gemm_kernel<HF, false, RT>), grid, dim3(SG_NT), smem, s, g);
+    if (src16) hipLaunchKernelGGL((style_gemm_kernel<HF, true, RT, RE>), grid, dim3(SG_NT), smem, s, g, rt);
+    else hipLaunchKernelGGL((style_gemm_kernel<HF, false, RT, RE>), grid, dim3(SG_NT), smem, s, g, rt);
   } else {
-    if (src16) hipLaunchKernelGGL((style_gemm_kernel<HB, true, RT>), grid, dim3(SG_NT), smem, s, g);
-    else hipLaunchKernelGGL((style_gemm_kernel<HB, false, RT>), grid, dim3(SG_NT), smem, s, g);
+    if (src16) hipLaunchKernelGGL((style_gemm_kernel<HB, true, RT, RE>), grid, dim3(SG_NT), smem, s, g, rt);
+    else hipLaunchKernelGGL((style_gemm_kernel<HB, false, RT, RE>), grid, dim3(SG_NT), smem, s, g, rt);
   }
   MDM_RETURN_IF_LAUNCH_FAILED();
   return MDM_OK;
 }
 
+bool style_gemm_route_supported(int D, int64_t M, int E, int hn_fmt, int h16) {
+  return style_gemm_supported(D, M) && (E == 8 || E == 16) && hn_fmt == h16 && (h16 == MDM_H16_BF16 || h16 == MDM_H16_F16) &&
+         style_gemm_route_parts(M) <= 1024;
+}
+int64_t style_gemm_route_parts(int64_t M) { return (M + 31) / 32; }
+
 int style_gemm(const void* src, int src_fmt, int64_t M, int D, int S, const float* pw, const float* pb, const float* sw, const float* sb,
                const float* sc, const int* pos4, const uint16_t* ws, const float* bias, const float* resid, float out_scale,
-               const float* colscale, float* out, uint16_t* out16, int h16, hipStream_t s) {
+               const float* colscale, float* out, uint16_t* out16, int h16, hipStream_t s, const StyleRoute* route) {
   if (M <= 0) return MDM_OK;
   if (!style_gemm_supported(D, M)) return MDM_ERR_UNSUPPORTED;
   if (!src || !sw || !sb || !sc || !ws || !bias || !out || S <= 0 || (pw && !pb)) return MDM_ERR_ARG;
@@ -436,7 +503,20 @@
   StyleGemmArgs g = {};
   g.src = src, g.M = M, g.S = S, g.pw = pw, g.pb = pb, g.sw = sw, g.sb = sb, g.sc = sc, g.pos4 = pos4, g.ws = ws, g.bias = bias;
   g.resid = resid, g.out_scale = out_scale, g.colscale = colscale, g.out = out, g.out16 = out16;
-  return launch_style_gemm<2>(g, src_fmt != 0, h16, s);
+  StyleRouteArgs rt = {};
+  if (route) {
+    if (!route->gate || !route->cursor) return MDM_ERR_ARG;
+    const MoeGateParams& p = *route->gate;
+    if (!style_gemm_route_supported(D, M, route->E, p.hn_bf16, h16)) return MDM_ERR_UNSUPPORTED;
+    if (!p.hn || !p.hist || !p.uimp || !p.top_idx || !p.top_val) return MDM_ERR_ARG;
+    for (int b = 0; b < 2; ++b)
+      if (!p.ln_w[b] || !p.ln_b[b] || !p.gate_w[b] || !p.gate_b[b] || ((uintptr_t)p.gate_w[b] & 15) || ((uintptr_t)p.ln_w[b] & 15) ||
+          ((uintptr_t)p.ln_b[b] & 15))
+        return MDM_ERR_ARG;
+    rt.p = p, rt.cursor = route->cursor;
+    return route->E == 8 ? launch_style_gemm<2, 8>(g, rt, src_fmt != 0, h16, s) : launch_style_gemm<2, 16>(g, rt, src_fmt != 0, h16, s);
+  }
+  return launch_style_gemm<2>(g, rt, src_fmt != 0, h16, s);
 }
 
 int64_t gemm_stream3_elems(int N, int K) { return (N == SG_D && K == SG_D) ? 2 * (int64_t)N * K + 16 * 512 : 0; }
```

After: 243.6 denoising-steps/sec, median of 6. 1.02x the previous value.
